# terran-project/terran

Hardware: AMD Instinct MI355X
Metric: frames/sec 1080p detect+embed+pose (higher is better)
Workload: dtype f16x3: operands x = hi + lo (two IEEE halfs, 22 bits), 3 f16 MFMAs per product, f32 accumulate; float32-grade results; 1 GPU; BASELINE configs[4]: 1080p detect+embed+pose; Detection(short_side=416) + Recognition(top-2) + Estimation(short_side=184); 32 frames per GPU per step resident in HBM; random-init weights; precision=f16x3, frames_per_gpu_step=32, faces_per_frame=2, resident_batch_reused=True, batches_in_flight_per_gpu=2

## Files before the change

### include/terran_amd.h

```cpp
#ifndef TERRAN_AMD_H
#define TERRAN_AMD_H

#include <stddef.h>
#include <stdint.h>

#ifdef __cplusplus
extern "C" {
#endif

#define TA_OK 0
#define TA_E_INVALID (-1)
#define TA_E_DEVICE (-2)
#define TA_E_CAPACITY (-3)
#define TA_E_OVERFLOW (-4)
#define TA_E_RANGE (-5)

#define TA_MODEL_RETINAFACE 1
#define TA_MODEL_ARCFACE 2
#define TA_MODEL_OPENPOSE 3

typedef struct ta_ctx ta_ctx;
typedef struct ta_model ta_model;
typedef struct ta_frames ta_frames;

// ... 260 lines not shown

int ta_jpeg_encode_header(int h, int w, int quality, int subsampling, uint8_t* out, size_t capacity, size_t* size);
int ta_jpeg_encode(ta_ctx* ctx, const ta_frames* frames, int quality, int subsampling, const uint8_t** out,
                   size_t* sizes);
int ta_jpeg_encode_last_stats(const ta_ctx* ctx, double* ms, int64_t* counts);
int ta_jpeg_encode_opt(ta_ctx* ctx, const ta_frames* frames, int quality, int subsampling, int optimize,
                       const uint8_t** out, size_t* sizes);
int ta_jpeg_optimal_table(const int64_t* freq, uint8_t* bits, uint8_t* vals, int* nvals);
int ta_jpeg_encode_last_opt_stats(const ta_ctx* ctx, double* ms);

int ta_model_load(ta_ctx* ctx, int kind, const void* blob, size_t bytes, ta_model** out);
int ta_program_check(int kind, const void* blob, size_t bytes, char* msg, size_t msg_capacity);
void ta_model_free(ta_model* m);
int ta_model_kind(const ta_model* m);

int ta_model_forward_frames(ta_model* m, const ta_frames* frames);
int ta_model_forward_crops(ta_model* m, const uint8_t* crops_nchw_bgr, int n);
int ta_model_tensor_shape(ta_model* m, int tensor, int* n, int* c, int* h, int* w);
int ta_model_read_tensor(ta_model* m, int tensor, int ch_off, int ch, float* dst_nchw);

int ta_model_tensor_unscale(const ta_model* m, int tensor, float* out, int capacity);
int ta_model_debug_amax(ta_model* m, int enable, float* out, int capacity);
int ta_model_graph_probe(ta_model* m, int reps, double* out_ms);

int ta_retinaface_run(ta_model* m, const ta_frames* frames, float score_thr, float nms_thr,
                      int capacity, int32_t* counts, float* boxes, float* landmarks, float* scores,
                      int32_t* required);
int ta_retinaface_postprocess(ta_ctx* ctx, const float* const heads[9], int n, int h, int w,
                              float score_thr, float nms_thr, int capacity, int32_t* counts,
                              float* boxes, float* landmarks, float* scores, int32_t* required);

int ta_arcface_embed_crops(ta_model* m, const uint8_t* crops_nchw_bgr, int n, int normalize, float* out);
int ta_arcface_embed_faces(ta_model* m, const ta_frames* frames, const int32_t* frame_index,
                           const double* inv_affine, int n, int normalize, float* out,
                           uint8_t* crops_out);
int ta_arcface_embed_faces_multi(ta_model* m, const ta_frames* const* frames, int n_sources, const int32_t* source_index,
                                 const int32_t* frame_index, const double* inv_affine, int n, int normalize,
                                 float* out, uint8_t* crops_out);
int ta_cosine_distance(ta_ctx* ctx, const float* a, int na, const float* b, int nb, int dim, float* out);

typedef struct ta_gallery ta_gallery;
int ta_gallery_create(ta_ctx* ctx, int dim, int64_t reserve_rows, ta_gallery** out);
void ta_gallery_free(ta_gallery* g);
int ta_gallery_add(ta_gallery* g, const float* rows, const int32_t* ids, int64_t n, int normalize);
int ta_gallery_remove(ta_gallery* g, const int32_t* ids, int n, int64_t* removed);
int ta_gallery_clear(ta_gallery* g);
int ta_gallery_size(const ta_gallery* g, int64_t* rows, int64_t* live);
int ta_gallery_download(const ta_gallery* g, float* rows_out, int32_t* ids_out);
int ta_gallery_search(ta_gallery* g, const float* queries, int nq, int k, int normalize, int32_t* out_row, int32_t* out_id,
                      float* out_dist);
int ta_gallery_cluster(ta_gallery* g, float threshold, int min_samples, int32_t* labels_out, int32_t* degree_out,
                       int32_t* n_clusters, int32_t* rounds);

int ta_openpose_run(ta_model* m, const ta_frames* frames, double scale, int capacity,
                    int32_t* counts, int32_t* keypoints, double* scores, int32_t* required);
int ta_openpose_group(ta_ctx* ctx, const float* pafs, const float* heatmaps, int n, int h, int w,
                      double scale, int capacity, int32_t* counts, int32_t* keypoints,
                      double* scores, int32_t* required);
int ta_openpose_last_stats(const ta_ctx* ctx, int64_t* peaks, int64_t* connections);

int ta_openpose_debug_read(ta_ctx* ctx, int n, int cap_peaks, int32_t* peak_counts, int32_t* peaks_yx,
                           float* peak_scores, int cap_conn, int32_t* conn_counts, int32_t* conn_ij,
                           float* conn_scores);
int ta_openpose_debug_capacity(ta_ctx* ctx, int n, int32_t* peak_capacity);

int ta_bicubic_x8(ta_ctx* ctx, const float* maps, int n, int c, int h, int w, float* out);

#define TA_CONV_AUTO 0
#define TA_CONV_GENERIC 1
#define TA_CONV_PIPE64 2
#define TA_CONV_PIPE128 3
#define TA_CONV_SPLIT_2x2 4
#define TA_CONV_SPLIT_2x2_P8 5
#define TA_CONV_SPLIT_2x4 6
#define TA_CONV_SPLIT_1x4 7
#define TA_CONV_WIN_2x2 8
#define TA_CONV_WIN_2x4 9
#define TA_CONV_WIN_1x4 10
#define TA_CONV_SPLIT_1x4_W2 11
#define TA_CONV_SPLIT_2x2_W2 12
int ta_debug_conv_variant(ta_ctx* ctx, int variant);
int ta_debug_range_check(ta_ctx* ctx);
int ta_debug_conv_counts(ta_ctx* ctx, int64_t* counts16, int reset);
int ta_debug_kernel_work(ta_ctx* ctx, char* csv, size_t capacity, int reset);

#ifdef __cplusplus
}
#endif
#endif
```

### terran_amd/csrc/conv_common.h

```cpp
#pragma once
#include <stdio.h>

#include "act_format.h"
#include "ta_internal.h"

#ifdef TA_CONV_TRACE
static __device__ __attribute__((unused)) long long ta_trace_buf[64];
#define TA_STAMP(i)                                                              \
  do {                                                                           \
    if (blockIdx.x == (unsigned)p.trace_block && (threadIdx.x & 63) == 0) ta_trace_buf[(i)] = __builtin_readcyclecounter(); \
  } while (0)
#define TA_TRACE_READER(name)                                                                   \
  extern "C" int name(long long* out, int n) {                                                  \
    return (int)hipMemcpyFromSymbol(out, HIP_SYMBOL(ta_trace_buf), sizeof(long long) * n);      \
  }
#else
#define TA_STAMP(i) do { } while (0)
#define TA_TRACE_READER(name)
#endif

typedef float f32x16 __attribute__((ext_vector_type(16)));
typedef float f32x4 __attribute__((ext_vector_type(4)));
typedef __bf16 bf16x8 __attribute__((ext_vector_type(8)));
typedef _Float16 f16x8 __attribute__((ext_vector_type(8)));

enum { PREC_F32 = 0, PREC_BF16X3 = 1, PREC_BF16 = 2, PREC_F16X3 = 3, PREC_F16 = 4, PREC_F16X2 = 5 };
__host__ __device__ constexpr bool prec_x3(int prec) { return prec == PREC_BF16X3 || prec == PREC_F16X3; }
__host__ __device__ constexpr bool prec_x2(int prec) { return prec == PREC_F16X2; }
__host__ __device__ constexpr bool prec_half(int prec) { return prec == PREC_F16X3 || prec == PREC_F16 || prec == PREC_F16X2; }
__host__ __device__ constexpr int prec_nmma(int prec) { return prec_x3(prec) ? 3 : (prec_x2(prec) ? 2 : 1); }

template <int PREC>
__device__ __forceinline__ f32x16 ta_mfma16(const bf16x8& a, const bf16x8& b, const f32x16& c) {
  if constexpr (prec_half(PREC))
    return __builtin_amdgcn_mfma_f32_32x32x16_f16(__builtin_bit_cast(f16x8, a), __builtin_bit_cast(f16x8, b), c, 0, 0, 0);
  else
    return __builtin_amdgcn_mfma_f32_32x32x16_bf16(a, b, c, 0, 0, 0);
}
template <int PREC>
__device__ __forceinline__ __bf16 ta_to16(float x) {
  if constexpr (prec_half(PREC)) return __builtin_bit_cast(__bf16, (_Float16)x);
  else return (__bf16)x;
}
template <int PREC>
__device__ __forceinline__ float ta_from16(__bf16 h) {
  if constexpr (prec_half(PREC)) return (float)__builtin_bit_cast(_Float16, h);
  else return (float)h;
}

#define LDS_PTR(p) ((__attribute__((address_space(3))) void*)(p))
#define GLB_PTR(p) ((const __attribute__((address_space(1))) void*)(p))

__device__ __forceinline__ void ta_dma16(const char* ubase, unsigned lane_off, const float* lds_dst) {
  const unsigned ldsa = (unsigned)(size_t)LDS_PTR(lds_dst);
  asm volatile("s_mov_b32 m0, %2\n\ts_nop 0\n\tglobal_load_lds_dwordx4 %0, %1" ::"v"(lane_off), "s"(ubase), "s"(ldsa)
               : "memory", "m0");
}

__device__ __forceinline__ int ta_xcd_tile(int n_pt, int xcd, int local) {
  const int base = n_pt >> 3, rem = n_pt & 7;
  if (local >= base + (xcd < rem ? 1 : 0)) return -1;
  return xcd * base + (xcd < rem ? xcd : rem) + local;
}

#define TA_INTERIOR 5
__device__ __forceinline__ int ta_border_class(int y, int x, int Ho, int Wo) {
  const int cy = Ho == 1 ? 3 : (y == 0 ? 0 : (y == Ho - 1 ? 2 : 1));
  const int cx = Wo == 1 ? 3 : (x == 0 ? 0 : (x == Wo - 1 ? 2 : 1));
  return cy * 4 + cx;
}

#define TA_F16_MAX_BITS 0x477FE000u
__device__ __forceinline__ unsigned ta_absbits(float x) { return __float_as_uint(x) & 0x7FFFFFFFu; }
__device__ __forceinline__ unsigned ta_amax4(unsigned m, const f32x4& v) {
  return max(max(m, max(ta_absbits(v[0]), ta_absbits(v[1]))), max(ta_absbits(v[2]), ta_absbits(v[3])));
}
__device__ __forceinline__ void ta_range_report(const ta_conv_launch& p, unsigned amax) {
  if (amax > TA_F16_MAX_BITS) *p.range_flag = 1;
  if (p.amax_index >= 0 && amax) atomicMax((unsigned*)p.range_flag + TA_AMAX_SLOT0 + 2 * p.amax_index, amax);
}
__device__ __forceinline__ float ta_relu(float v) { return v < 0.f ? 0.f : v; }

template <int WM_TILES, int WN_TILES>
__device__ __forceinline__ void conv_epilogue(const ta_conv_launch& p, f32x16 (&acc)[WM_TILES][WN_TILES], int co_tile0,
// ... 55 lines not shown
    if (p.act == TA_ACT_RELU) {
#pragma unroll
      for (int a = 0; a < WM_TILES; ++a)
#pragma unroll
        for (int j = 0; j < 4; ++j)
#pragma unroll
          for (int e = 0; e < 4; ++e) v[a][j][e] = ta_relu(v[a][j][e]);
    } else if (p.act == TA_ACT_PRELU) {
#pragma unroll
      for (int a = 0; a < WM_TILES; ++a)
#pragma unroll
        for (int j = 0; j < 4; ++j)
#pragma unroll
          for (int e = 0; e < 4; ++e) v[a][j][e] = v[a][j][e] > 0.f ? v[a][j][e] : v[a][j][e] * slope[a][j][e];
    }
    if (p.res) {
      const int ry = p.res_up2 ? (y >> 1) : y, rx = p.res_up2 ? (x >> 1) : x;
      const float* rs = p.res + (size_t)img * p.res_img + (size_t)ry * p.res_row + (size_t)rx * p.res_pix + p.res_off0;
      f32x4 r4[WM_TILES][4];
#pragma unroll
      for (int a = 0; a < WM_TILES; ++a)
#pragma unroll
        for (int j = 0; j < 4; ++j) {
          const int co = co_base + a * 32 + 8 * j;
          r4[a][j] = ta_ld4(rs, p.res_ch + (co < co_max ? co : co_max), p.res_fmt);
        }
#pragma unroll
      for (int a = 0; a < WM_TILES; ++a)
#pragma unroll
        for (int j = 0; j < 4; ++j)
#pragma unroll
          for (int e = 0; e < 4; ++e) v[a][j][e] += r4[a][j][e];
    }
    float* o = p.out + (size_t)img * p.out_img + (size_t)y * p.out_row + (size_t)x * p.out_pix + p.out_off0;
    if (pix_ok) {
#pragma unroll
      for (int a = 0; a < WM_TILES; ++a)
#pragma unroll
        for (int j = 0; j < 4; ++j) {
          const int co = co_base + a * 32 + 8 * j;
          if (co < p.cout) {
            ta_st4(o, p.out_ch + co, p.out_fmt, v[a][j]);
            if (p.range_check) amax = ta_amax4(amax, v[a][j]);
          }
        }
    }
    if (p.out2) {
      float* o2 = p.out2 + (size_t)img * p.o2_img + (size_t)y * p.o2_row + (size_t)x * p.o2_pix + p.o2_off0;
      f32x4 sc[WM_TILES][4], sh[WM_TILES][4];
#pragma unroll
      for (int a = 0; a < WM_TILES; ++a)
#pragma unroll
        for (int j = 0; j < 4; ++j) {
          sc[a][j] = *(const f32x4*)(p.scale2 + co_base + a * 32 + 8 * j);
          sh[a][j] = *(const f32x4*)(p.shift2 + co_base + a * 32 + 8 * j);
        }
      if (pix_ok) {
#pragma unroll
        for (int a = 0; a < WM_TILES; ++a)
#pragma unroll
          for (int j = 0; j < 4; ++j) {
            const int co = co_base + a * 32 + 8 * j;
            f32x4 z;
#pragma unroll
            for (int e = 0; e < 4; ++e) z[e] = v[a][j][e] * sc[a][j][e] + sh[a][j][e];
            if (co < p.cout) {
              ta_st4(o2, p.o2_ch + co, p.o2_fmt, z);
              if (p.range_check) amax = ta_amax4(amax, z);
            }
          }
      }
    }
  }
  ta_range_report(p, amax);
}

struct ta_k_walk {
  int cb, kx, ky, b_off, a_slab;
  int cblocks, kw, kh, pix_bytes, row_bytes;
  __device__ __forceinline__ ta_k_walk(const ta_conv_launch& p, int s0) {
    cblocks = p.k_cblocks;
    kw = p.k_w;
    kh = p.k_h;
    pix_bytes = p.in_pix * 4;
    row_bytes = p.in_row * 4;
    if (s0 == 0) {
      cb = kx = ky = b_off = a_slab = 0;
      return;
    }
    const int taps = kw * kh;
    cb = s0 / taps;
    const int tap = s0 - cb * taps;
    ky = tap / kw;
    kx = tap - ky * kw;
    b_off = cb * 128 + kx * pix_bytes + ky * row_bytes;
    a_slab = tap * cblocks + cb;
  }
  __device__ __forceinline__ void advance() {
    ++kx;
    b_off += pix_bytes;
    a_slab += cblocks;
    if (kx == kw) {
      kx = 0;
      b_off += row_bytes - kw * pix_bytes;
      if (++ky == kh) {
        ky = 0;
        ++cb;
        b_off += 128 - kh * row_bytes;
        a_slab = cb;
      }
    }
  }
};

__device__ __forceinline__ int ta_div_r(int t, int d, float rd, int fast) {
  if (!fast) return t / d;
  int q = (int)((float)t * rd);
  const int r = t - q * d;
  if (r < 0) --q;
  else if (r >= d) ++q;
  return q;
}

struct ta_pixel_walk {
  int img0, y0, x0, Wo, Ho;
  float rWo, rHo;
  __device__ __forceinline__ ta_pixel_walk(const ta_conv_launch& p, int pt0, int HoWo) {
    Wo = p.Wo;
    Ho = p.Ho;
    if (p.fast_div) {
      img0 = ta_div_r(pt0, HoWo, p.r_HoWo, 1);
      const int rem = pt0 - img0 * HoWo;
      y0 = ta_div_r(rem, Wo, p.r_Wo, 1);
      x0 = rem - y0 * Wo;
      rWo = p.r_Wo;
      rHo = p.r_Ho;
      return;
    }
    img0 = pt0 / HoWo;
    const int rem = pt0 - img0 * HoWo;
    y0 = rem / p.Wo;
    x0 = rem - y0 * p.Wo;
    rWo = 1.0f / (float)p.Wo;
    rHo = 1.0f / (float)p.Ho;
  }
  static __device__ __forceinline__ void divmod(int t, int d, float rd, int& q, int& r) {
    q = (int)((float)t * rd);
    r = t - q * d;
    if (r < 0) {
      --q;
      r += d;
    } else if (r >= d) {
      ++q;
      r -= d;
    }
  }
  __device__ __forceinline__ void at(int d, int& img, int& y, int& x) const {
    int qy, qi;
    divmod(x0 + d, Wo, rWo, qy, x);
    divmod(y0 + qy, Ho, rHo, qi, y);
    img = img0 + qi;
  }
};

struct ta_f32x8 {
  f32x4 a, b;
};
__device__ __forceinline__ ta_f32x8 ta_ld8(const float* pix, int ch, int fmt) {
  ta_f32x8 r;
  if (fmt == TA_FMT_F32) {
    r.a = *(const f32x4*)(pix + ch);
    r.b = *(const f32x4*)(pix + ch + 4);
    return r;
  }
  if (fmt == TA_FMT_F16) {
    const uint4 w = *(const uint4*)((const char*)pix + 2 * ch);
    float v[8];
    ta_unpack2<true>(w.x, v[0], v[1]);
    ta_unpack2<true>(w.y, v[2], v[3]);
    ta_unpack2<true>(w.z, v[4], v[5]);
    ta_unpack2<true>(w.w, v[6], v[7]);
    r.a = f32x4{v[0], v[1], v[2], v[3]};
    r.b = f32x4{v[4], v[5], v[6], v[7]};
    return r;
  }
  const char* q = (const char*)pix + ta_split_chan(ch);
  const uint4 h = *(const uint4*)q, l = *(const uint4*)(q + 64);
  const unsigned hw[4] = {h.x, h.y, h.z, h.w}, lw[4] = {l.x, l.y, l.z, l.w};
  float v[8];
#pragma unroll
  for (int i = 0; i < 4; ++i) {
    float h0, h1, l0, l1;
    if (fmt == TA_FMT_SPLIT16) {
      ta_unpack2<true>(hw[i], h0, h1);
      ta_unpack2<true>(lw[i], l0, l1);
    } else {
// ... 387 lines not shown
        const int c = ((wm * WM_TILES + a) * 32 + 8 * j + 4 * (lane >> 5)) >> 2;
        *(f32x4*)(lds + (row * NCH + (c ^ (row & (NCH - 1)))) * 4) =
            f32x4{acc[a][b][4 * j], acc[a][b][4 * j + 1], acc[a][b][4 * j + 2], acc[a][b][4 * j + 3]};
      }
  }
  __syncthreads();
  if (tid == 0) TA_STAMP(22);
  conv_epilogue_drain<BN, BM, 256>(p, lds, ct0, pt0, tid, HoWo, 0);
}

template <int WM_TILES, int WN_TILES, int PREC>
__device__ __forceinline__ void conv_slab_mma(const float* st, f32x16 (&acc)[WM_TILES][WN_TILES], int a_row0, int b_row0, int fsw,
                                              int fcb, int lane) {
  if constexpr (PREC == PREC_F32) {
#pragma unroll
    for (int g = 0; g < 4; ++g) {
      const int pc = ((fcb + g) ^ fsw) * 4;
      f32x4 av[WM_TILES], bv[WN_TILES];
#pragma unroll
      for (int a = 0; a < WM_TILES; ++a) av[a] = *(const f32x4*)(st + (a_row0 + a * 32) * 32 + pc);
#pragma unroll
      for (int b = 0; b < WN_TILES; ++b) bv[b] = *(const f32x4*)(st + (b_row0 + b * 32) * 32 + pc);
#pragma unroll
      for (int e = 0; e < 4; ++e)
#pragma unroll
        for (int a = 0; a < WM_TILES; ++a)
#pragma unroll
          for (int b = 0; b < WN_TILES; ++b)
            acc[a][b] = __builtin_amdgcn_mfma_f32_32x32x2f32(av[a][e], bv[b][e], acc[a][b], 0, 0, 0);
    }
  } else {
    const int kg = lane >> 5;
#pragma unroll
    for (int t = 0; t < 2; ++t) {
      bf16x8 ah[WM_TILES], al[WM_TILES], bh[WN_TILES], bl[WN_TILES];
#pragma unroll
      for (int a = 0; a < WM_TILES; ++a) {
        ah[a] = *(const bf16x8*)(st + (a_row0 + a * 32) * 32 + ((2 * kg + t) ^ fsw) * 4);
        if constexpr (prec_x3(PREC) || prec_x2(PREC)) al[a] = *(const bf16x8*)(st + (a_row0 + a * 32) * 32 + ((4 + 2 * kg + t) ^ fsw) * 4);
      }
#pragma unroll
      for (int b = 0; b < WN_TILES; ++b) {
        const f32x4 x0 = *(const f32x4*)(st + (b_row0 + b * 32) * 32 + ((fcb + 2 * t) ^ fsw) * 4);
        const f32x4 x1 = *(const f32x4*)(st + (b_row0 + b * 32) * 32 + ((fcb + 2 * t + 1) ^ fsw) * 4);
#pragma unroll
        for (int e = 0; e < 4; ++e) {
          const __bf16 h0 = ta_to16<PREC>(x0[e]), h1 = ta_to16<PREC>(x1[e]);
          bh[b][e] = h0;
          bh[b][4 + e] = h1;
          if constexpr (prec_x3(PREC)) {
            bl[b][e] = ta_to16<PREC>(x0[e] - ta_from16<PREC>(h0));
            bl[b][4 + e] = ta_to16<PREC>(x1[e] - ta_from16<PREC>(h1));
          }
        }
      }
      if constexpr (prec_x3(PREC) || prec_x2(PREC)) {
#pragma unroll
        for (int a = 0; a < WM_TILES; ++a)
#pragma unroll
          for (int b = 0; b < WN_TILES; ++b)
            acc[a][b] = ta_mfma16<PREC>(al[a], bh[b], acc[a][b]);
      }
      if constexpr (prec_x3(PREC)) {
#pragma unroll
        for (int a = 0; a < WM_TILES; ++a)
#pragma unroll
          for (int b = 0; b < WN_TILES; ++b)
            acc[a][b] = ta_mfma16<PREC>(ah[a], bl[b], acc[a][b]);
      }
#pragma unroll
      for (int a = 0; a < WM_TILES; ++a)
#pragma unroll
        for (int b = 0; b < WN_TILES; ++b)
          acc[a][b] = ta_mfma16<PREC>(ah[a], bh[b], acc[a][b]);
    }
  }
}

struct ta_tile_grid {
  int n_ct, n_pt, groups;
  ta_tile_grid(const ta_conv_launch& p, int BN, int BM) : n_ct(p.coutp / BN), n_pt((p.M + BM - 1) / BM), groups(((n_pt + 7) / 8) * n_ct) {}
};

#define TA_NOTE_KERNEL(ctx, ...)                                    \
  do {                                                              \
    static char _name[80];                                          \
    if (!_name[0]) snprintf(_name, sizeof(_name), __VA_ARGS__);     \
    (ctx)->note_kernel(_name);                                      \
  } while (0)
```

### terran_amd/csrc/conv_igemm.hip

```cpp
#include <string.h>

#include "conv_common.h"

static bool is_split_variant(int v) {
  return v == TA_CV_SPLIT_2x2 || v == TA_CV_SPLIT_2x2_P8 || v == TA_CV_SPLIT_2x4 || v == TA_CV_SPLIT_1x4 || v == TA_CV_SPLIT_1x4_W2 || v == TA_CV_SPLIT_2x2_W2;
}

static bool variant_eligible(int v, const ta_conv_launch& p) {
  const bool split_in = p.in_fmt == ta_split_fmt_of(p.prec);
  const bool deep = p.uniform_k && (p.n_slabs >= 2 || p.prec == PREC_F16);
  const bool staged = ((p.out_ch | p.res_ch | p.o2_ch) & 7) == 0 && (p.cout & 3) == 0;
  switch (v) {
    case TA_CV_GENERIC: return p.in_fmt == TA_FMT_F32 && !p.group_cout;
    case TA_CV_PIPE64: return deep && staged && p.coutp % 64 == 0 && !p.group_cout && (p.in_fmt == TA_FMT_F32 || (split_in && p.prec != PREC_F16));
    case TA_CV_PIPE128: return deep && staged && p.coutp % 128 == 0 && !p.group_cout && p.in_fmt == TA_FMT_F32;
    case TA_CV_SPLIT_2x2:
    case TA_CV_SPLIT_2x2_P8:
    case TA_CV_SPLIT_2x4: return deep && split_in && staged && p.coutp % 128 == 0;
    case TA_CV_SPLIT_1x4: return deep && split_in && staged && p.coutp % 64 == 0 && (!p.group_cout || p.group_cout % 64 == 0);
    case TA_CV_SPLIT_2x2_W2: return deep && split_in && staged && p.coutp % 128 == 0 && p.k_split <= 1;
    case TA_CV_SPLIT_1x4_W2: return deep && split_in && staged && p.coutp % 64 == 0 && (!p.group_cout || p.group_cout % 64 == 0) && p.k_split <= 1;
    case TA_CV_WIN_2x2:
    case TA_CV_WIN_2x4:
    case TA_CV_WIN_1x4: {
      const bool base = deep && split_in && staged && (p.prec == PREC_F16X3 || p.prec == PREC_F16X2) && p.stride == 1 && !p.pool && p.k_split <= 1 &&
                        p.k_w * p.k_h >= 4 && p.n_slabs == p.k_w * p.k_h * p.k_cblocks;
      if (!base) return false;
      if (v == TA_CV_WIN_1x4) return p.coutp % 64 == 0 && (!p.group_cout || p.group_cout % 64 == 0) && ta_win_patch_rows(p, 256) <= TA_WIN_PR_1x4;
      if (p.coutp % 128) return false;
      return v == TA_CV_WIN_2x2 ? ta_win_patch_rows(p, 128) <= TA_WIN_PR_2x2 : ta_win_patch_rows(p, 256) <= TA_WIN_PR_2x4;
    }
  }
  return false;
}

static int choose_variant_streamed(const ta_conv_launch& p);
static int choose_variant(const ta_conv_launch& p) {
  const int v = choose_variant_streamed(p);
  const int w = v == TA_CV_SPLIT_2x2 ? TA_CV_WIN_2x2 : (v == TA_CV_SPLIT_2x4 ? TA_CV_WIN_2x4 : (v == TA_CV_SPLIT_1x4 ? TA_CV_WIN_1x4 : 0));
  return (w && variant_eligible(w, p)) ? w : v;
}
static int choose_variant_streamed(const ta_conv_launch& p) {
  if (p.uniform_k && (p.n_slabs >= 2 || p.prec == PREC_F16)) {
    if (variant_eligible(TA_CV_SPLIT_2x2, p)) {
      if (p.prec != PREC_F32 && p.k_split == 1) {
        const int n_ct = p.coutp / 128;
        const int t1 = ((p.M + 127) / 128) * n_ct, t2 = ((p.M + 255) / 256) * n_ct;
        const int r1 = (t1 + 255) / 256, r2 = (t2 + 255) / 256;
        if (r2 * 184 < r1 * 100) return TA_CV_SPLIT_2x4;
      }
      return TA_CV_SPLIT_2x2;
    }
    if (variant_eligible(TA_CV_SPLIT_1x4, p)) {
      constexpr int W2_SLABS = 18, W2_TILES = 1024;
      if (p.prec != PREC_F32 && p.n_slabs <= W2_SLABS && (p.M + 255) / 256 * (p.coutp / 64) >= W2_TILES && variant_eligible(TA_CV_SPLIT_1x4_W2, p))
        return TA_CV_SPLIT_1x4_W2;
      return TA_CV_SPLIT_1x4;
    }
    if (variant_eligible(TA_CV_PIPE64, p)) return TA_CV_PIPE64;
  }
  return TA_CV_GENERIC;
}

static int launch_variant(ta_ctx* ctx, int v, const ta_conv_launch& p) {
  switch (v) {
    case TA_CV_GENERIC:
    case TA_CV_PIPE64:
    case TA_CV_PIPE128: return ta_launch_conv_sym(ctx, v, p);
    case TA_CV_SPLIT_2x2:
    case TA_CV_SPLIT_2x2_P8:
    case TA_CV_SPLIT_2x4:
    case TA_CV_SPLIT_1x4:
    case TA_CV_SPLIT_1x4_W2:
    case TA_CV_SPLIT_2x2_W2:
    case TA_CV_WIN_2x2:
    case TA_CV_WIN_2x4:
    case TA_CV_WIN_1x4: return ta_launch_conv_split(ctx, v, p);
  }
  return ta_fail(ctx, TA_E_INVALID, "conv: unknown kernel variant %d", v);
}

int ta_launch_conv(ta_ctx* ctx, const ta_conv_launch& p_in, double flops) {
  if (p_in.M <= 0) return TA_OK;
  ta_conv_launch p = p_in;
#ifdef TA_CONV_TRACE
  p.trace_block = ctx->conv_trace_block;
#endif
  if (p.k_split < 1 || !p.partial) p.k_split = 1;
  if (p.coutp % 32 != 0 || p.cout % 4 != 0) return ta_fail(ctx, TA_E_INVALID, "conv: bad cout padding");
  if (p.prec != PREC_F32 && p.prec != PREC_BF16X3 && p.prec != PREC_BF16 && p.prec != PREC_F16X3 && p.prec != PREC_F16 && p.prec != PREC_F16X2)
    return ta_fail(ctx, TA_E_INVALID, "conv: unknown precision mode %d", p.prec);
  if (p.in_fmt != TA_FMT_F32 && p.in_fmt != ta_split_fmt_of(p.prec))
    return ta_fail(ctx, TA_E_INVALID, "conv: input tensor format %d does not belong to precision mode %d", p.in_fmt, p.prec);
  p.range_flag = ctx->range_flag;
  int v = p.variant;
  if (v != TA_CV_AUTO) {
    if (!variant_eligible(v, p))
      return ta_fail(ctx, TA_E_INVALID, "conv: forced kernel variant %d cannot run this layer (cin-uniform %d, slabs %d, coutp %d, "
                     "input format %d, groups %d)", v, p.uniform_k, p.n_slabs, p.coutp, p.in_fmt, p.group_cout ? 1 : 0);
  } else {
    const bool prefer = ctx->conv_force && variant_eligible(ctx->conv_force, p) && (!p.pool || is_split_variant(ctx->conv_force));
    v = prefer ? ctx->conv_force : choose_variant(p);
    if (!variant_eligible(v, p)) return ta_fail(ctx, TA_E_INVALID, "conv: pre-split input reached a kernel that cannot read it");
  }
  const bool is_split = is_split_variant(v);
  if (!is_split || v == TA_CV_SPLIT_1x4_W2 || v == TA_CV_SPLIT_2x2_W2) p.k_split = 1;
  if (p.pool) {
    if (!is_split || p.res || p.out2 || (p.out_ch & 7) || (p.M & 3) || (p.act != TA_ACT_RELU && p.act != TA_ACT_NONE))
      return ta_fail(ctx, TA_E_INVALID, "conv: the fused max-pool needs the split-role kernel and a plain epilogue (variant %d)", v);
    p.k_split = 1;
  }
  ctx->conv_counts[v] += 1;
  ctx->cur_flops = flops;
  ta_prof_scope scope(ctx, 0, flops);
  return launch_variant(ctx, v, p);
}

extern "C" {

int ta_debug_conv_variant(ta_ctx* ctx, int variant) {
  if (!ctx || variant < 0 || variant >= TA_CV_COUNT) return TA_E_INVALID;
  ctx->conv_force = variant;
  return TA_OK;
}

int ta_debug_kernel_work(ta_ctx* ctx, char* csv, size_t capacity, int reset) {
  if (!ctx || (!csv && capacity)) return TA_E_INVALID;
  std::string out;
  for (const auto& kv : ctx->kernel_work) {
    char line[200];
    const auto t = ctx->kernel_ms.find(kv.first);
    snprintf(line, sizeof(line), "%s;%lld;%.6e;%.6f\n", kv.first.c_str(), (long long)kv.second.first, kv.second.second,
             t == ctx->kernel_ms.end() ? 0.0 : t->second);
    out += line;
  }
  if (reset) {
    ta_drain_profile(ctx);
    ctx->kernel_work.clear();
    ctx->kernel_ms.clear();
  }
  if (out.size() + 1 > capacity) return ta_fail(ctx, TA_E_CAPACITY, "kernel_work: %zu bytes needed", out.size() + 1);
  memcpy(csv, out.c_str(), out.size() + 1);
  return TA_OK;
}

int ta_debug_conv_counts(ta_ctx* ctx, int64_t* counts16, int reset) {
  if (!ctx) return TA_E_INVALID;
  for (int i = 0; i < TA_CV_COUNT; ++i) {
    if (counts16) counts16[i] = ctx->conv_counts[i];
    if (reset) ctx->conv_counts[i] = 0;
  }
  return TA_OK;
}

}
```

### terran_amd/csrc/conv_split_kernels.h

```cpp
#pragma once
#include "conv_common.h"

__device__ __forceinline__ void split_acc_clear(f32x16 (&acc)[2][2]) {
#pragma unroll
  for (int a = 0; a < 2; ++a)
#pragma unroll
    for (int b = 0; b < 2; ++b)
#pragma unroll
      for (int r = 0; r < 16; ++r) acc[a][b][r] = 0.f;
}

template <int PREC>
__device__ __forceinline__ void split_mma16(f32x16 (&acc)[2][2], const bf16x8 (&ah)[2], const bf16x8 (&al)[2], const bf16x8 (&bh)[2],
                                            const bf16x8 (&bl)[2]) {
  if constexpr (prec_x3(PREC) || prec_x2(PREC)) {
#pragma unroll
    for (int a = 0; a < 2; ++a)
#pragma unroll
      for (int b = 0; b < 2; ++b) acc[a][b] = ta_mfma16<PREC>(al[a], bh[b], acc[a][b]);
  }
  if constexpr (prec_x3(PREC)) {
#pragma unroll
    for (int a = 0; a < 2; ++a)
#pragma unroll
      for (int b = 0; b < 2; ++b) acc[a][b] = ta_mfma16<PREC>(ah[a], bl[b], acc[a][b]);
  }
  if constexpr (PREC == PREC_F16) {
#pragma unroll
    for (int a = 0; a < 2; ++a)
#pragma unroll
      for (int b = 0; b < 2; ++b) acc[a][b] = ta_mfma16<PREC>(al[a], bl[b], acc[a][b]);
  }
#pragma unroll
  for (int a = 0; a < 2; ++a)
#pragma unroll
    for (int b = 0; b < 2; ++b) acc[a][b] = ta_mfma16<PREC>(ah[a], bh[b], acc[a][b]);
}

template <int NREAD, int NMMA>
__device__ __forceinline__ void split_pin() {
#pragma unroll
  for (int i = 0; i < NREAD; ++i) {
    __builtin_amdgcn_sched_group_barrier(0x100, 1, 0);
    __builtin_amdgcn_sched_group_barrier(0x008, 1, 0);
  }
  __builtin_amdgcn_sched_group_barrier(0x008, NMMA - NREAD, 0);
}


template <int CM, int CN, int NP, int PREC, int STAGES>
__global__ __launch_bounds__(64 * (CM * CN + NP), STAGES == 2 ? 4 : (CM * CN + NP) / 4) void conv_igemm_split(const ta_conv_launch p) {
  static_assert(NP == 4 || NP == 8, "4 or 8 producer waves");
  static_assert(STAGES == 3 || (STAGES == 2 && CM * CN == 4 && NP == 4), "3-stage ring, or the 2-stage two-workgroups-per-CU variant of the 8-wave tiles");
  static_assert(CM * CN == 4 || CM * CN == 8, "consumer grid: 1x4 (64 cout x 256 px), 2x2 (128 x 128) or 2x4 (128 x 256)");
  constexpr int NC = CM * CN;
  constexpr int BN = CM * 64, BM = CN * 64;
  constexpr int NI = (BN + BM) / 8 / NP;
  constexpr int QA = BN / 8 / NP;
  constexpr int STAGE = (BN + BM) * 32;
  extern __shared__ __attribute__((aligned(16))) float lds[];

  const int tid = threadIdx.x;
  const int lane = tid & 63;
  const int wave = __builtin_amdgcn_readfirstlane(tid >> 6);
  if (wave == 0) TA_STAMP(0);
  if (wave == NC) TA_STAMP(8);

  const int n_ct = p.coutp / BN;
  const int n_pt = (p.M + BM - 1) / BM;
  const int tile_blocks = (((n_pt + 7) >> 3) * n_ct) << 3;
  const int ks = p.k_split > 1 ? ta_div_r(blockIdx.x, tile_blocks, p.r_tile_blocks, p.fast_div) : 0;
  const int bid = blockIdx.x - ks * tile_blocks;
  const int grp = bid >> 3, xcd = bid & 7;
  const int gq = ta_div_r(grp, n_ct, p.r_nct, p.fast_div);
  const int pt = ta_xcd_tile(n_pt, xcd, gq);
  if (pt < 0) return;
  const int ct0 = (grp - gq * n_ct) * BN;
  const int pt0 = pt * BM;
  const int HoWo = p.Ho * p.Wo;
  int s_begin = 0, S = p.n_slabs;
  if (p.k_split > 1) {
    s_begin = (int)(((long long)ks * p.n_slabs) / p.k_split);
    S = (int)(((long long)(ks + 1) * p.n_slabs) / p.k_split) - s_begin;
  }

  if (wave >= NC) {
    const int pw = wave - NC;
    const int pchunk = lane & 7;
    const int lchunk = pchunk ^ ((4 * (pw & 1) + (lane >> 4)) & 7);
    const char* a_base = (const char*)p.w;
    const size_t a_slab_bytes = (size_t)p.coutp * 128;
    unsigned a_off[QA];
    unsigned b_off[NI - QA];
#pragma unroll
    for (int q = 0; q < QA; ++q) a_off[q] = (unsigned)(((ct0 + (q * NP + pw) * 8 + (lane >> 3)) * 32 + lchunk * 4) * 4);
    ta_k_walk wa(p, s_begin);
    auto issue_a = [&](int, int stage) {
#pragma unroll
      for (int q = 0; q < QA; ++q) ta_dma16(a_base + (size_t)wa.a_slab * a_slab_bytes, a_off[q], lds + stage * STAGE + (q * NP + pw) * 256);
      wa.advance();
    };
    issue_a(0, 0);
    if (S > 1) issue_a(1, 1);
    const int pl = p.pool;
    const ta_pixel_walk walk(p, pl ? pt0 >> 2 : pt0, HoWo);
    const int in_ch = p.in_ch_off + (p.group_cout ? (ct0 / p.group_cout) * p.group_cin : 0);
    const size_t off0 = (size_t)walk.img0 * p.in_img + (size_t)((walk.y0 << pl) * p.stride) * p.in_row +
                        (size_t)((walk.x0 << pl) * p.stride) * p.in_pix + p.in_off0 + in_ch;
    const char* b_base = (const char*)(p.in + off0);
    ta_k_walk wb(p, s_begin);
#pragma unroll
    for (int q = QA; q < NI; ++q) {
      const int d = (q * NP + pw) * 8 + (lane >> 3) - BN;
      int img, y, x;
      const int dd = pt0 + d < p.M ? d : 0;
      walk.at(pl ? dd >> 2 : dd, img, y, x);
      if (pl) {
        y = 2 * y + ((dd >> 1) & 1);
        x = 2 * x + (dd & 1);
      }
      const size_t off = (size_t)img * p.in_img + (size_t)(y * p.stride) * p.in_row + (size_t)(x * p.stride) * p.in_pix +
                         p.in_off0 + in_ch;
      b_off[q - QA] = (unsigned)((off - off0) * 4 + lchunk * 16);
      ta_dma16(b_base + wb.b_off, b_off[q - QA], lds + (q * NP + pw) * 256);
    }
    wb.advance();
    auto issue_b = [&](int stage) {
#pragma unroll
      for (int q = QA; q < NI; ++q) ta_dma16(b_base + wb.b_off, b_off[q - QA], lds + stage * STAGE + (q * NP + pw) * 256);
      wb.advance();
    };
    if (wave == NC) TA_STAMP(9);
    if (S > 1) issue_b(1);
    if (wave == NC) TA_STAMP(10);
    int stage = STAGES == 2 ? 0 : 2;
    if constexpr (STAGES == 2) {
      for (int s = 0; s < S; ++s) {
        if (s == 0 && S > 1) asm volatile("s_waitcnt vmcnt(%0)" ::"n"(NI - QA) : "memory");
        else asm volatile("s_waitcnt vmcnt(0)" ::: "memory");
        __builtin_amdgcn_s_barrier();
        asm volatile("" ::: "memory");
        if (s >= 1 && s + 1 < S) {
          issue_a(s + 1, stage);
          issue_b(stage);
          stage ^= 1;
        }
      }
    } else
    for (int s = 0; s < S; ++s) {
      if (s == 0 && S > 1) asm volatile("s_waitcnt vmcnt(%0)" ::"n"(NI - QA) : "memory");
      else if (s + 1 < S) asm volatile("s_waitcnt vmcnt(%0)" ::"n"(NI) : "memory");
      else asm volatile("s_waitcnt vmcnt(0)" ::: "memory");
      __builtin_amdgcn_s_barrier();
      asm volatile("" ::: "memory");
      if (s + 2 < S) {
        issue_a(s + 2, stage);
        issue_b(stage);
        stage = stage == 2 ? 0 : stage + 1;
      }
    }
    {
      __builtin_amdgcn_s_barrier();
      __builtin_amdgcn_s_barrier();
      asm volatile("" ::: "memory");
      bool done = false;
      if constexpr (PREC != PREC_F32) done = conv_drain_dispatch<BN, BM, 64 * (NC + NP), (PREC == PREC_F16 ? 2 : (prec_half(PREC) ? 1 : 0))>(p, lds, ct0, pt0, tid, HoWo);
      if (!done) conv_epilogue_drain<BN, BM, 64 * (NC + NP)>(p, lds, ct0, pt0, tid, HoWo, ks);
    }
    return;
  }

  const int cm = wave / CN, cn = wave % CN;
  int stage = 0;
  f32x16 acc[2][2];
  split_acc_clear(acc);
  const int frow = lane & 31;
  const int fsw = (frow >> 1) & 7;
  const int kg = lane >> 5;
  const int a_row0 = cm * 64 + frow;
  const int b_row0 = BN + cn * 64 + frow;
  struct Frag {
    bf16x8 ah[2], al[2], bh[2], bl[2];
    f32x4 a32[2][2], b32[2][2];
  };
  const int fcb = kg * 4;
  auto load = [&](Frag& f, const float* st, int t) {
    if constexpr (PREC == PREC_F32) {
#pragma unroll
      for (int g = 0; g < 2; ++g) {
        const int pc = ((fcb + 2 * t + g) ^ fsw) * 4;
#pragma unroll
        for (int a = 0; a < 2; ++a) f.a32[a][g] = *(const f32x4*)(st + (a_row0 + a * 32) * 32 + pc);
#pragma unroll
        for (int b = 0; b < 2; ++b) f.b32[b][g] = *(const f32x4*)(st + (b_row0 + b * 32) * 32 + pc);
      }
      return;
    }
#pragma unroll
    for (int a = 0; a < 2; ++a) {
      f.ah[a] = *(const bf16x8*)(st + (a_row0 + a * 32) * 32 + ((2 * kg + t) ^ fsw) * 4);
      if constexpr (prec_x3(PREC) || prec_x2(PREC) || PREC == PREC_F16) f.al[a] = *(const bf16x8*)(st + (a_row0 + a * 32) * 32 + ((4 + 2 * kg + t) ^ fsw) * 4);
    }
#pragma unroll
    for (int b = 0; b < 2; ++b) {
      f.bh[b] = *(const bf16x8*)(st + (b_row0 + b * 32) * 32 + ((2 * kg + t) ^ fsw) * 4);
      if constexpr (prec_x3(PREC) || PREC == PREC_F16) f.bl[b] = *(const bf16x8*)(st + (b_row0 + b * 32) * 32 + ((4 + 2 * kg + t) ^ fsw) * 4);
    }
  };
  auto mma = [&](const Frag& f) {
    if constexpr (PREC == PREC_F32) {
#pragma unroll
      for (int g = 0; g < 2; ++g)
#pragma unroll
// ... 205 lines not shown
      pb[b] = (unsigned)buf * (unsigned)(PATCH * 4) + row * 128u + ((((unsigned)(2 * kg)) ^ ((row >> 1) & 7u)) << 4);
    }
  };
  auto load = [&](Frag& f, const float* st, int t) {
#pragma unroll
    for (int a = 0; a < 2; ++a) {
      f.ah[a] = *(const bf16x8*)(st + (a_row0 + a * 32) * 32 + ((2 * kg + t) ^ fsw) * 4);
      f.al[a] = *(const bf16x8*)(st + (a_row0 + a * 32) * 32 + ((4 + 2 * kg + t) ^ fsw) * 4);
    }
#pragma unroll
    for (int b = 0; b < 2; ++b) {
      const char* q = (const char*)patch0 + (pb[b] ^ (unsigned)(t << 4));
      f.bh[b] = *(const bf16x8*)q;
      if constexpr (prec_x3(PREC)) f.bl[b] = *(const bf16x8*)((const char*)patch0 + ((pb[b] ^ (unsigned)(t << 4)) ^ 64u));
    }
  };
  auto mma = [&](const Frag& f) { split_mma16<PREC>(acc, f.ah, f.al, f.bh, f.bl); };
  constexpr int NREAD = prec_x3(PREC) ? 8 : 6;
  constexpr int NMMA = prec_x3(PREC) ? 12 : 8;
  int kx = 0, ky = 0, cb = 0, tap_off = 0, stage = 0;
  Frag F0, F1;
  baddr(0, 0);
  if (wave == 0) TA_STAMP(1);
  __builtin_amdgcn_s_barrier();
  asm volatile("" ::: "memory");
  if (wave == 0) TA_STAMP(2);
  load(F0, lds, 0);
  for (int g = 0; g + 1 < S; ++g) {
    const float* st = lds + stage * A_STAGE;
    stage = stage == 2 ? 0 : stage + 1;
    __builtin_amdgcn_sched_barrier(0);
    load(F1, st, 1);
    mma(F0);
    split_pin<NREAD, NMMA>();
    __builtin_amdgcn_sched_barrier(0);
    if (++kx == p.k_w) {
      kx = 0;
      tap_off += wp - p.k_w;
      if (++ky == p.k_h) {
        ky = 0;
        ++cb;
        tap_off = -1;
      }
    }
    ++tap_off;
    asm volatile("s_waitcnt lgkmcnt(0)" ::: "memory");
    baddr(tap_off, cb & 1);
    __builtin_amdgcn_s_barrier();
    asm volatile("" ::: "memory");
    load(F0, lds + stage * A_STAGE, 0);
    mma(F1);
    split_pin<NREAD, NMMA>();
    __builtin_amdgcn_sched_barrier(0);
  }
  load(F1, lds + stage * A_STAGE, 1);
  mma(F0);
  mma(F1);
  if (wave == 0) TA_STAMP(3);
  {
    __builtin_amdgcn_s_barrier();
    asm volatile("" ::: "memory");
    if (wave == 0) TA_STAMP(5);
    conv_epilogue_park<BN>(acc, lds, cm, cn, lane);
    if (wave == 0) TA_STAMP(6);
    asm volatile("s_waitcnt lgkmcnt(0)" ::: "memory");
    __builtin_amdgcn_s_barrier();
    asm volatile("" ::: "memory");
    if (wave == 0) TA_STAMP(7);
    if (!conv_drain_dispatch<BN, BM, 64 * (NC + NP), 1>(p, lds, ct0, pt0, tid, HoWo))
      conv_epilogue_drain<BN, BM, 64 * (NC + NP)>(p, lds, ct0, pt0, tid, HoWo, 0);
  }
  if (wave == 0) TA_STAMP(4);
}

static void split_launch_facts(ta_ctx* ctx, ta_conv_launch& q, const ta_tile_grid& g, int BM, int split_fmt, bool lean_ok) {
  q.r_nct = 1.0f / (float)g.n_ct;
  q.r_tile_blocks = 1.0f / (float)(g.groups * 8);
  q.r_Wo = 1.0f / (float)q.Wo;
  q.r_Ho = 1.0f / (float)q.Ho;
  q.r_HoWo = 1.0f / (float)(q.Ho * q.Wo);
  const long long grid = (long long)g.groups * 8 * q.k_split;
  q.fast_div = (grid < (1 << 24) && (long long)q.M + BM < (1 << 24)) ? 1 : 0;
  const long long n_img = q.Ho * q.Wo > 0 ? ((long long)q.M + q.Ho * q.Wo - 1) / (q.Ho * q.Wo) : 0;
  auto fits = [&](long long img_stride, int off0) { return ((n_img + 1) * img_stride + off0) * 4 < (1LL << 32); };
  bool ok = lean_ok && q.out_fmt == split_fmt && (q.cout & 7) == 0 && ((q.out_ch | q.res_ch | q.o2_ch) & 7) == 0 && fits(q.out_img, q.out_off0);
  if (q.res) ok = ok && q.res_fmt == split_fmt && fits(q.res_img, q.res_off0);
  if (q.out2) ok = ok && q.o2_fmt == split_fmt && fits(q.o2_img, q.o2_off0);
  const bool plain = !q.res && !q.out2;
  ok = ok && (q.pool ? (plain && q.act == TA_ACT_RELU) : (q.bias9 ? (plain && q.act == TA_ACT_PRELU) : (plain || (q.res && q.act == TA_ACT_NONE))));
  q.fast_drain = ok ? 1 : 0;
  if (ok) ctx->conv_counts[TA_CV_COUNT - 1] += 1;
}

template <int CM, int CN, int NP, int PREC, int STAGES>
static int launch_split(ta_ctx* ctx, const ta_conv_launch& p) {
  constexpr int BN = CM * 64, BM = CN * 64;
  const ta_tile_grid g(p, BN, BM);
  const size_t lds_bytes = (size_t)STAGES * (BN + BM) * 32 * sizeof(float);
  auto kern = conv_igemm_split<CM, CN, NP, PREC, STAGES>;
  TA_SET_LDS_ATTR(ctx, kern, lds_bytes);
  ta_conv_launch q = p;
  constexpr int SPLIT_FMT = PREC == PREC_F16 ? TA_FMT_F16 : (prec_half(PREC) ? TA_FMT_SPLIT16 : TA_FMT_SPLIT);
  split_launch_facts(ctx, q, g, BM, SPLIT_FMT, PREC != PREC_F32 && p.k_split == 1);
  TA_NOTE_KERNEL(ctx, "conv_igemm_split<%d,%d,%d,%d,%d>", CM, CN, NP, PREC, STAGES);
  hipLaunchKernelGGL(kern, dim3(g.groups * 8 * p.k_split), dim3(64 * (CM * CN + NP)), lds_bytes, ctx->stream, q);
  TA_HIP(ctx, hipGetLastError());
  return TA_OK;
}

template <int CM, int CN, int PREC, int PR>
static int launch_win(ta_ctx* ctx, const ta_conv_launch& p) {
  constexpr int BN = CM * 64, BM = CN * 64;
  const ta_tile_grid g(p, BN, BM);
  constexpr size_t ring = (size_t)(3 * BN + 2 * PR) * 128, park = (size_t)BM * BN * 4;
  constexpr size_t lds_bytes = ring > park ? ring : park;
  static_assert(lds_bytes <= 160 * 1024, "one workgroup's LDS");
  auto kern = conv_igemm_win<CM, CN, PREC, PR>;
  TA_SET_LDS_ATTR(ctx, kern, lds_bytes);
  ta_conv_launch q = p;
  q.k_split = 1;
  split_launch_facts(ctx, q, g, BM, TA_FMT_SPLIT16, true);
  TA_NOTE_KERNEL(ctx, "conv_igemm_win<%d,%d,%d,%d>", CM, CN, PREC, PR);
  hipLaunchKernelGGL(kern, dim3(g.groups * 8), dim3(64 * (CM * CN + 4)), lds_bytes, ctx->stream, q);
  TA_HIP(ctx, hipGetLastError());
  return TA_OK;
}

template <int PREC>
static int launch_split_variant(ta_ctx* ctx, int v, const ta_conv_launch& p) {
  switch (v) {
    case TA_CV_SPLIT_2x2: return launch_split<2, 2, 4, PREC, 3>(ctx, p);
    case TA_CV_SPLIT_2x2_P8: return launch_split<2, 2, 8, PREC, 3>(ctx, p);
    case TA_CV_SPLIT_2x4: return launch_split<2, 4, 4, PREC, 3>(ctx, p);
    case TA_CV_SPLIT_1x4: return launch_split<1, 4, 4, PREC, 3>(ctx, p);
    case TA_CV_SPLIT_1x4_W2: return launch_split<1, 4, 4, PREC, 2>(ctx, p);
    case TA_CV_SPLIT_2x2_W2: return launch_split<2, 2, 4, PREC, 2>(ctx, p);
    case TA_CV_WIN_2x2:
    case TA_CV_WIN_2x4:
    case TA_CV_WIN_1x4:
      if constexpr (PREC == PREC_F16X3 || PREC == PREC_F16X2) {
        if (v == TA_CV_WIN_2x2) return launch_win<2, 2, PREC, TA_WIN_PR_2x2>(ctx, p);
        if (v == TA_CV_WIN_2x4) return launch_win<2, 4, PREC, TA_WIN_PR_2x4>(ctx, p);
        return launch_win<1, 4, PREC, TA_WIN_PR_1x4>(ctx, p);
      }
      break;
  }
  return ta_fail(ctx, TA_E_INVALID, "conv: unknown kernel variant %d", v);
}
```

### terran_amd/csrc/model_load.hip

```cpp
#include <stdarg.h>
#include <string.h>

#include "act_format.h"
#include "ta_internal.h"

namespace {
struct refusal {
  char* msg;
  size_t cap;
  int operator()(const char* fmt, ...) const {
    if (msg && cap) {
      va_list ap;
      va_start(ap, fmt);
      vsnprintf(msg, cap, fmt, ap);
      va_end(ap);
    }
    return TA_E_INVALID;
  }
};
const int MAX_DIM = 1 << 24;
bool within(int v, int lo, int hi) { return v >= lo && v <= hi; }
}

int ta_program_parse(int kind, const void* blob, size_t bytes, ta_program* out, char* msg, size_t msg_capacity) {
  const refusal no{msg, msg_capacity};
  if (msg && msg_capacity) msg[0] = 0;
  if (!blob || !out) return no("model blob: null pointer");
  if (bytes < sizeof(ta_blob_header)) return no("model blob too small");
  ta_blob_header& h = out->hdr;
  memcpy(&h, blob, sizeof(h));
  if (h.magic != TA_BLOB_MAGIC || h.version != 9) return no("model blob: bad magic/version (this library reads version 9)");
  if (h.kind != kind) return no("model blob is kind %d, expected %d", h.kind, kind);
  if (h.n_tensors <= 0 || h.n_ops <= 0 || h.n_outputs < 0 || h.n_outputs > 16 || h.input_tensor < 0 ||
      h.input_tensor >= h.n_tensors)
    return no("model blob: bad counts");
  auto inside = [&](int64_t off, int64_t count, size_t each) {
    return off >= 0 && count >= 0 && (uint64_t)off <= bytes && (uint64_t)count <= (bytes - (size_t)off) / each;
  };
  if (!inside(h.tensors_off, h.n_tensors, sizeof(ta_tensor_desc))) return no("model blob: truncated (tensor table)");
  if (!inside(h.ops_off, h.n_ops, sizeof(ta_op_desc))) return no("model blob: truncated (op table)");
  if (!inside(h.weights_off, h.weights_bytes, 1)) return no("model blob: truncated (weights)");
  const int T = h.n_tensors;
  std::vector<ta_tensor_desc>& td = out->tdesc;
  std::vector<ta_op_desc>& ops = out->ops;
  td.resize(T);
  ops.resize(h.n_ops);
  memcpy(td.data(), (const char*)blob + h.tensors_off, T * sizeof(ta_tensor_desc));
  memcpy(ops.data(), (const char*)blob + h.ops_off, h.n_ops * sizeof(ta_op_desc));
  auto bad_w = [&](int64_t off, size_t need) { return off >= 0 && (uint64_t)off + need > (uint64_t)h.weights_bytes; };

  for (int t = 0; t < T; ++t) {
    const ta_tensor_desc& d = td[t];
    if (!within(d.channels, 1, MAX_DIM) || !within(d.halo, 0, 1024) || !within(d.alias_of, -2, T - 1) || d.alias_of == t)
      return no("model blob: malformed tensor %d", t);
    if ((d.fmt != TA_FMT_F32 && d.channels % 32) || (d.fmt == TA_FMT_F16 && d.channels % 64) || d.fmt < 0 || d.fmt > TA_FMT_F16)
      return no("model blob: tensor %d: format %d with %d channels", t, d.fmt, d.channels);
    if (d.unscale_off >= 0 && (t == h.input_tensor || (d.unscale_off & 3) || bad_w(d.unscale_off, (size_t)d.channels * sizeof(float))))
      return no("model blob: inconsistent activation scales (tensor %d)", t);
  }
  for (int i = 0; i < h.n_outputs; ++i)
    if (!within(h.outputs[i], 0, T - 1)) return no("model blob: output %d is tensor %d, out of range", i, h.outputs[i]);

  std::vector<char> set(T, 0);
  set[h.input_tensor] = 1;
  auto view_ready = [&](int id) {
    const int src = td[id].alias_of;
    if (src >= 0 && !set[id]) set[id] = set[src];
    return src < 0 || set[id];
  };
  std::vector<int> writer_lane(T, 0), reader_lanes(T, 0);

  for (int oi = 0; oi < h.n_ops; ++oi) {
    const ta_op_desc& op = ops[oi];
    auto bad_t = [&](int t) { return t < 0 || t >= T; };
    const char* why = nullptr;
    auto need = [&](bool ok, const char* what) {
      if (!ok && !why) why = what;
    };
    need(!bad_t(op.in) && !bad_t(op.out) && (op.res < 0 || !bad_t(op.res)) && (op.out2 < 0 || !bad_t(op.out2)), "tensor index out of range");
    need(within(op.kh, 1, 64) && within(op.kw, 1, 64) && within(op.stride, 1, 64) && within(op.pad, 0, 64) && within(op.cin, 0, MAX_DIM) &&
             within(op.cout, 0, MAX_DIM) && within(op.coutp, 0, MAX_DIM) && within(op.n_slabs, 0, MAX_DIM) && within(op.groups, 0, 1 << 16) &&
             within(op.in_ch_off, 0, MAX_DIM) && within(op.out_ch_off, 0, MAX_DIM) && within(op.res_ch_off, 0, MAX_DIM) &&
             within(op.out2_ch_off, 0, MAX_DIM),
         "field out of range");
    if (why) return no("model blob: malformed op %d: %s", oi, why);
    const size_t row = (size_t)op.coutp * 4, image = (size_t)op.n_slabs * op.coutp * 128;
    const bool wus_ok = !bad_w(op.bias_off, row) && op.wus_off == op.bias_off + 4 * (int64_t)op.coutp && !bad_w(op.wus_off, row);
    if (op.type == TA_OP_CONV) {
      need(op.w_off >= 0 && op.bias_off >= 0, "no weights or no bias");
      need(op.cin % 4 == 0 && op.cout % 4 == 0 && op.coutp % 32 == 0 && op.n_slabs > 0, "channel counts or K slabs");
      need(op.prec >= 0 && op.prec <= 5, "arithmetic mode");
      need(!bad_w(op.w_off, image), "w_off past the weight region");
      need(!bad_w(op.bias_off, row), "bias_off past the weight region");
      need(!bad_w(op.prelu_off, row), "prelu_off past the weight region");
      need(!bad_w(op.scale2_off, row), "scale2_off past the weight region");
      need(!bad_w(op.shift2_off, row), "shift2_off past the weight region");
      need(wus_ok, "wus_off is not the [coutp] floats behind the bias");
      need(op.act != TA_ACT_PRELU || op.prelu_off >= 0, "PReLU without slopes");
      need(op.out2 < 0 || (op.scale2_off >= 0 && op.shift2_off >= 0), "second output without its affine");
      need(!ta_op_border_bias(op) || !(op.out2 >= 0 || op.scale2_off < 0 || op.kh != 3 || op.kw != 3 || op.stride != 1 || op.pad != 1 ||
                                       op.pool || bad_w(op.scale2_off, 16 * row)),
           "border-bias table on a conv that is not a plain 3x3, stride 1, pad 1");
    } else if (op.type == TA_OP_RFSTEM) {
      need(op.w_off >= 0 && (op.cout == 16 || op.cout == 32), "front op without weights or with another width than 16 / 32");
      need(!bad_w(op.w_off, (op.cout == 32 ? 448 + 704 : 448) * 4), "w_off past the weight region");
    } else if (op.type == TA_OP_DWPW) {
      need(op.w_off >= 0 && op.bias_off >= 0 && op.scale2_off >= 0 && op.shift2_off >= 0, "no weights or no bias");
      need(op.cin % 4 == 0 && op.cout % 4 == 0 && op.coutp % 32 == 0 && op.n_slabs > 0 && (int64_t)op.n_slabs * 32 >= op.cin && op.stride <= 2,
           "channel counts, K slabs or stride");
      need(op.prec == 0 || op.prec == 3, "arithmetic mode");
      need(!bad_w(op.w_off, image), "w_off past the weight region");
      need(!bad_w(op.bias_off, row), "bias_off past the weight region");
      need(!bad_w(op.scale2_off, (size_t)op.cin * 36), "scale2_off past the weight region");
      need(!bad_w(op.shift2_off, (size_t)op.cin * 4), "shift2_off past the weight region");
      need(wus_ok, "wus_off is not the [coutp] floats behind the bias");
    } else if (op.type == TA_OP_DWCONV) {
      need(op.w_off >= 0 && op.bias_off >= 0 && op.cin % 4 == 0 && op.kh == 3 && op.kw == 3, "no weights, no bias, or not 3x3");
      need(!bad_w(op.w_off, (size_t)op.cin * 36), "w_off past the weight region");
      need(!bad_w(op.bias_off, (size_t)op.cin * 4), "bias_off past the weight region");
    } else if (op.type != TA_OP_MAXPOOL && op.type != TA_OP_COPYCH) {
      return no("model blob: unknown op type %d (op %d)", op.type, oi);
    }
    if (why) return no("model blob: malformed op %d: %s", oi, why);

    const ta_tensor_desc &ti = td[op.in], &to = td[op.out];
    if (!view_ready(op.in)) return no("model blob: alias tensor %d used before its source %d (op %d)", op.in, ti.alias_of, oi);
    if (!set[op.in]) return no("model blob: op %d reads unset tensor %d", oi, op.in);
    if (op.type != TA_OP_CONV && (ti.fmt == TA_FMT_F16 || to.fmt == TA_FMT_F16))
      return no("model blob: op %d: only convs read and write half-float tensors", oi);
    if ((op.type == TA_OP_CONV || op.type == TA_OP_DWCONV) && ti.halo < op.pad)
      return no("model blob: op %d needs halo %d, tensor has %d", oi, op.pad, ti.halo);
    if (op.type == TA_OP_CONV) {
      const ta_k_geometry kg = ta_conv_k_geometry(op, ti.fmt);
      if (op.groups > 1 && !(kg.uniform && op.n_slabs >= 2 && op.cout % op.groups == 0 && (op.cout / op.groups) % 128 == 0 && op.cout == op.coutp &&
                             op.in_ch_off % 32 == 0 && op.in_ch_off + (int64_t)op.groups * op.cin <= ti.channels && ti.fmt == ta_split_fmt_of(op.prec)))
        return no("model blob: op %d: unsupported grouped convolution", oi);
      if (op.pool && (op.out2 >= 0 || op.res >= 0 || op.groups > 1 || op.cin % 32 || op.coutp % 64))
        return no("model blob: op %d: unsupported conv + max-pool fusion", oi);
      if (ti.fmt == TA_FMT_F16 && (!kg.uniform || op.in_ch_off || op.groups > 1 || op.prec != 4))
        return no("model blob: op %d: a half-float tensor feeds whole-tensor convs of the f16 mode only", oi);
      if (ti.fmt != TA_FMT_F16 && (int64_t)op.kh * op.kw * (op.cin / 4) > (int64_t)op.n_slabs * 8)
        return no("model blob: op %d has too few K slabs", oi);
    } else if (op.type == TA_OP_DWCONV) {
      if (op.in_ch_off || op.out_ch_off) return no("model blob: op %d: depthwise conv on a channel slice is not supported", oi);
      if (ti.unscale_off >= 0 || to.unscale_off >= 0) return no("model blob: inconsistent activation scales (op %d)", oi);
    } else if (op.type == TA_OP_RFSTEM) {
      if (oi != 0 || op.in != h.input_tensor || ti.alias_of != -2)
        return no("model blob: the RetinaFace front op must be op 0 on a shape-only input tensor (op %d)", oi);
    } else if (op.type == TA_OP_DWPW) {
      if (ti.halo < 1) return no("model blob: op %d (dw+pw) needs an input halo", oi);
      if (ti.fmt != TA_FMT_F32 || op.in_ch_off || op.cin > ti.channels) return no("model blob: op %d: unsupported dw+pw block", oi);
    }
    set[op.out] = 1;
    if (op.out2 >= 0) set[op.out2] = 1;

    const int lane = ta_op_lane(op);
    bool shared = lane == 3 || (lane && (op.type != TA_OP_CONV || ta_op_packed_ksplit(op) > 1 || op.pool));
    for (int t : {op.in, op.res}) {
      if (t < 0) continue;
      if (writer_lane[t] && writer_lane[t] != lane) shared = true;
      reader_lanes[t] |= 1 << lane;
    }
    for (int t : {op.out, op.out2}) {
      if (t < 0) continue;
      if (reader_lanes[t] & ~(1 << lane)) shared = true;
      if (writer_lane[t] && writer_lane[t] != lane) shared = true;
      if (lane) writer_lane[t] = lane;
      else if (reader_lanes[t] >> 1) shared = true;
    }
    if (shared) return no("model blob: an op lane (side stream) shares tensors with ops outside it (op %d)", oi);
  }
  for (int t = 0; t < T; ++t)
    if (!view_ready(t)) return no("model blob: alias tensor %d used before its source %d", t, td[t].alias_of);
  return TA_OK;
}

extern "C" {

int ta_program_check(int kind, const void* blob, size_t bytes, char* msg, size_t msg_capacity) {
  ta_program p;
  return ta_program_parse(kind, blob, bytes, &p, msg, msg_capacity);
}

int ta_model_load(ta_ctx* ctx, int kind, const void* blob, size_t bytes, ta_model** out) {
  ta_enter(ctx);
  if (!ctx || !blob || !out) return TA_E_INVALID;
  *out = nullptr;
  std::unique_ptr<ta_model> m(new ta_model());
  char why[256];
  if (ta_program_parse(kind, blob, bytes, m.get(), why, sizeof(why)) != TA_OK) return ta_fail(ctx, TA_E_INVALID, "%s", why);
  const ta_blob_header& h = m->hdr;
  const char* weights = (const char*)blob + h.weights_off;
  m->ctx = ctx;
  m->kind = kind;
  m->unscale_host.resize(h.n_tensors);
  for (int t = 0; t < h.n_tensors; ++t)
    if (m->tdesc[t].unscale_off >= 0) {
      const float* v = (const float*)(weights + m->tdesc[t].unscale_off);
      m->unscale_host[t].assign(v, v + m->tdesc[t].channels);
    }
  m->tensor_read.assign(h.n_tensors, 0);
  for (auto& op : m->ops) {
    m->tensor_read[op.in] = 1;
    if (op.res >= 0) m->tensor_read[op.res] = 1;
    if ((op.type == TA_OP_CONV || op.type == TA_OP_DWPW) && (op.prec == 3 || op.prec == 4 || op.prec == 5)) m->has_half_ops = true;
  }
  for (int t = 0; t < h.n_tensors; ++t) {
    const int src = m->tdesc[t].alias_of;
// ... 34 lines not shown
```

### terran_amd/csrc/model_plan.hip

```cpp
#include <algorithm>

#include "act_format.h"
#include "ta_internal.h"

#define TA_MAX_PLANS 4
#define TA_MAX_PLAN_BYTES ((size_t)96 << 30)

static int conv_out(int in, int k, int stride, int pad) { return (in + 2 * pad - k) / stride + 1; }

static void activate(ta_model* m, ta_plan* pl, int n_run) {
  m->active = pl;
  pl->last_use = ++m->use_counter;
  m->run_n = n_run;
}

static int plan_capacity(int kind, int n) {
  if (kind != TA_MODEL_ARCFACE) return n;
  if (n <= 8) return 8;
  if (n <= 32) return 32;
  return (n + 63) / 64 * 64;
}

static int infer_shapes(const ta_model* m, int h, int w, std::vector<ta_tensor>& ts, std::vector<bool>& set) {
  ta_ctx* ctx = m->ctx;
// ... 21 lines not shown
    set[id] = true;
    return TA_OK;
  };

  for (const ta_op_desc& op : m->ops) {
    TA_TRY(resolve_alias(op.in));
    const ta_tensor& ti = ts[op.in];
    switch (op.type) {
      case TA_OP_CONV:
      case TA_OP_DWCONV: {
        const int oh = conv_out(ti.h, op.kh, op.stride, op.pad), ow = conv_out(ti.w, op.kw, op.stride, op.pad);
        if (op.type == TA_OP_CONV && op.pool) {
          TA_TRY(set_out(op.out, oh / 2, ow / 2));
          break;
        }
        TA_TRY(set_out(op.out, oh, ow));
        if (op.type == TA_OP_CONV && op.out2 >= 0) TA_TRY(set_out(op.out2, oh, ow));
        break;
      }
      case TA_OP_MAXPOOL:
        TA_TRY(set_out(op.out, ti.h / 2, ti.w / 2));
        break;
      case TA_OP_RFSTEM:
        if (op.cout == 32)
          TA_TRY(set_out(op.out, ((ti.h + 1) / 2 + 1) / 2, ((ti.w + 1) / 2 + 1) / 2));
        else
          TA_TRY(set_out(op.out, (ti.h + 1) / 2, (ti.w + 1) / 2));
        break;
      case TA_OP_DWPW:
        TA_TRY(set_out(op.out, conv_out(ti.h, 3, op.stride, 1), conv_out(ti.w, 3, op.stride, 1)));
        break;
      case TA_OP_COPYCH:
        TA_TRY(set_out(op.out, ti.h, ti.w));
        break;
    }
  }
  for (size_t i = 0; i < ts.size(); ++i) TA_TRY(resolve_alias((int)i));
  return TA_OK;
}

int ta_model_plan(ta_model* m, int n_run, int h, int w) {
  ta_ctx* ctx = m->ctx;
  if (n_run <= 0 || h <= 0 || w <= 0) return ta_fail(ctx, TA_E_INVALID, "plan: bad input shape %dx%dx%d", n_run, h, w);
  const int n = plan_capacity(m->kind, n_run);
  auto fits = [&](const ta_plan* pl) { return pl && pl->n == n && pl->h == h && pl->w == w; };
  if (fits(m->active)) {
    activate(m, m->active, n_run);
    return TA_OK;
  }
  for (auto& pl : m->plans)
    if (fits(pl.get())) {
      activate(m, pl.get(), n_run);
      return TA_OK;
    }
  TA_HIP(ctx, hipStreamSynchronize(ctx->stream));
  for (;;) {
    size_t bytes = 0;
    for (auto& pl : m->plans) bytes += pl->arena_bytes;
    if (m->plans.size() < TA_MAX_PLANS && bytes <= TA_MAX_PLAN_BYTES) break;
    if (m->plans.empty()) break;
    size_t lru = 0;
    for (size_t i = 1; i < m->plans.size(); ++i)
      if (m->plans[i]->last_use < m->plans[lru]->last_use) lru = i;
    if (m->plans[lru].get() == m->active) m->active = nullptr;
    m->plans.erase(m->plans.begin() + lru);
  }
  std::unique_ptr<ta_plan> np(new ta_plan());
  np->n = n;
  np->h = h;
  np->w = w;

  const int T = m->hdr.n_tensors;
  std::vector<ta_tensor> ts(T);
  std::vector<bool> set(T, false);
  for (int i = 0; i < T; ++i) {
    ts[i].c = m->tdesc[i].channels;
    ts[i].halo = m->tdesc[i].halo;
    ts[i].fmt = m->tdesc[i].fmt;
    if (m->tdesc[i].unscale_off >= 0) {
      ts[i].unscale_dev = (const float*)(m->weights_dev + m->tdesc[i].unscale_off);
      ts[i].unscale_host = m->unscale_host[i].data();
    }
    ts[i].n = n;
  }
  TA_TRY(infer_shapes(m, h, w, ts, set));

  size_t total = 0;
  std::vector<size_t> offs(T, 0);
  for (int i = 0; i < T; ++i) {
    if (!set[i] || !ts[i].owns) continue;
    const size_t bytes = ts[i].elems() * sizeof(float);
    if (bytes >= ((size_t)1 << 32)) return ta_fail(ctx, TA_E_INVALID, "plan: tensor %d exceeds 4 GiB; split the batch", i);
    offs[i] = total;
    total += (bytes + 255) & ~(size_t)255;
  }
  size_t ws_bytes = 0;
  for (const ta_op_desc& op : m->ops) {
    if (op.type != TA_OP_CONV) continue;
    const int M = ts[op.out].n * ts[op.out].h * ts[op.out].w;
    const int ks = ta_op_ksplit(op, ts[op.in].fmt);
    if (ks > 1) ws_bytes = std::max(ws_bytes, (size_t)ks * M * op.coutp * sizeof(float));
  }
  const size_t ws_off = total;
  total += (ws_bytes + 255) & ~(size_t)255;
  hipError_t e = hipMalloc((void**)&np->arena, total ? total : 256);
  if (e != hipSuccess) {
    np->arena = nullptr;
    return ta_fail(ctx, TA_E_DEVICE, "plan: hipMalloc(%zu) failed: %s", total, hipGetErrorString(e));
  }
  np->arena_bytes = total;
  TA_HIP(ctx, hipMemsetAsync(np->arena, 0, total ? total : 256, ctx->stream));
  for (int i = 0; i < T; ++i)
    if (set[i] && ts[i].owns) ts[i].dev = (float*)(np->arena + offs[i]);
  for (int i = 0; i < T; ++i)
    if (set[i] && !ts[i].owns) ts[i].dev = m->tdesc[i].alias_of >= 0 ? ts[m->tdesc[i].alias_of].dev : nullptr;
  np->splitk_ws = ws_bytes ? (float*)(np->arena + ws_off) : nullptr;

  std::vector<int32_t> ktab;
  np->ktab_off.assign(m->ops.size(), 0);
  for (size_t oi = 0; oi < m->ops.size(); ++oi) {
    const ta_op_desc& op = m->ops[oi];
    if (op.type != TA_OP_CONV) continue;
    const ta_tensor& ti = ts[op.in];
    np->ktab_off[oi] = ktab.size();
    if (ti.fmt == TA_FMT_F16) continue;
    const int cpt = op.cin / 4;
    const int nq = op.kh * op.kw * cpt;
    for (int q = 0; q < op.n_slabs * 8; ++q) {
      int32_t off = 0;
      if (q < nq) {
        const int tap = q / cpt, ch = (q % cpt) * 4;
        const int ky = tap / op.kw, kx = tap % op.kw;
        off = (int32_t)((((size_t)ky * ti.wp() + kx) * ti.c + op.in_ch_off + ch) * sizeof(float));
      }
      ktab.push_back(off);
    }
  }
  if (!ktab.empty()) {
    TA_HIP(ctx, hipMalloc((void**)&np->ktab_dev, ktab.size() * sizeof(int32_t)));
    TA_HIP(ctx, hipMemcpy(np->ktab_dev, ktab.data(), ktab.size() * sizeof(int32_t), hipMemcpyHostToDevice));
  }
  TA_HIP(ctx, hipStreamSynchronize(ctx->stream));
  np->tensors.swap(ts);
  m->plans.push_back(std::move(np));
  activate(m, m->plans.back().get(), n_run);
  return TA_OK;
}
```

### terran_amd/csrc/model_run.hip

```cpp
#include <stdlib.h>
#include <string.h>

#include <algorithm>
#include <chrono>

#include "act_format.h"
#include "ta_internal.h"

static int conv_out(int in, int k, int stride, int pad) { return (in + 2 * pad - k) / stride + 1; }

static const float* wptr(const ta_model* m, int64_t off) { return off < 0 ? nullptr : (const float*)(m->weights_dev + off); }

static void put(const ta_strides& s, int& img, int& row, int& pix, int& off0) { img = s.img, row = s.row, pix = s.pix, off0 = s.off0; }

static void print_op_profile(ta_model* m, std::vector<hipEvent_t>& ev) {
  (void)hipStreamSynchronize(m->ctx->stream);
  double tot_ms = 0, tot_fl = 0;
  for (size_t oi = 0; oi < m->ops.size(); ++oi) {
    const ta_op_desc& op = m->ops[oi];
    const ta_tensor& to = m->tensor(op.out);
    float ms = 0.f;
    (void)hipEventElapsedTime(&ms, ev[2 * oi], ev[2 * oi + 1]);
    const ta_tensor& ti = m->tensor(op.in);
    const double M = op.type == TA_OP_CONV && op.pool
// ... 40 lines not shown
  const ta_plan& pl = *m->active;
  for (size_t oi = 0; oi < m->ops.size(); ++oi) {
    const ta_op_desc& op = m->ops[oi];
    const ta_tensor& ti = m->tensor(op.in);
    const ta_tensor& to = m->tensor(op.out);
    const int lane = lanes_on ? ta_op_lane(op) : 0;
    ctx->stream = lanes.main;
    if (lane) {
      const int li = lane - 1;
      if (!ctx->side_stream[li]) {
        TA_HIP(ctx, hipStreamCreateWithFlags(&ctx->side_stream[li], hipStreamNonBlocking));
        TA_HIP(ctx, hipEventCreateWithFlags(&ctx->side_fork[li], hipEventDisableTiming));
        TA_HIP(ctx, hipEventCreateWithFlags(&ctx->side_join[li], hipEventDisableTiming));
      }
      if (!lanes.started[li]) {
        TA_HIP(ctx, hipEventRecord(ctx->side_fork[li], lanes.main));
        TA_HIP(ctx, hipStreamWaitEvent(ctx->side_stream[li], ctx->side_fork[li], 0));
        lanes.started[li] = true;
      }
      ctx->stream = ctx->side_stream[li];
    }
    struct evp_t {
      hipEvent_t e;
      hipStream_t s;
      bool on;
      ~evp_t() { if (on) (void)hipEventRecord(e, s); }
    } evp{prof_ops ? ev[2 * oi + 1] : nullptr, ctx->stream, prof_ops};
    if (prof_ops) (void)hipEventRecord(ev[2 * oi], ctx->stream);
    switch (op.type) {
      case TA_OP_CONV: {
        ta_conv_launch p;
        memset(&p, 0, sizeof(p));
        p.in = ti.dev;
        p.w = wptr(m, op.w_off);
        p.ktab = pl.ktab_dev + pl.ktab_off[oi];
        p.bias = wptr(m, op.bias_off);
        p.prelu = wptr(m, op.prelu_off);
        p.out = to.dev;
        p.M = m->run_n * to.h * to.w;
        p.Ho = to.h;
        p.Wo = to.w;
        p.n_slabs = op.n_slabs;
        p.coutp = op.coutp;
        p.cout = op.cout;
        p.act = op.act;
        p.stride = op.stride;
        p.prec = op.prec;
        const ta_k_geometry kg = ta_conv_k_geometry(op, ti.fmt);
        p.uniform_k = kg.uniform;
        p.k_cblocks = kg.cblocks;
        p.k_w = op.kw;
        p.k_h = op.kh;
        p.in_ch_off = op.in_ch_off;
        put(ta_tensor_strides(ti, op.pad, false), p.in_img, p.in_row, p.in_pix, p.in_off0);
        p.win_wp = ti.wp();
        p.win_img = ti.hp() * ti.wp();
        put(ta_tensor_strides(to, 0, false), p.out_img, p.out_row, p.out_pix, p.out_off0);
        p.out_ch = op.out_ch_off;
        p.out_fmt = to.fmt;
        p.in_fmt = ti.fmt;
        if (op.res >= 0) {
          const ta_tensor& tr = m->tensor(op.res);
          p.res = tr.dev;
          put(ta_tensor_strides(tr, 0, false), p.res_img, p.res_row, p.res_pix, p.res_off0);
          p.res_ch = op.res_ch_off;
          p.res_fmt = tr.fmt;
          p.res_up2 = op.res_up2;
        }
        if (op.out2 >= 0) {
          const ta_tensor& t2 = m->tensor(op.out2);
          p.out2 = t2.dev;
          p.scale2 = wptr(m, op.scale2_off);
          p.shift2 = wptr(m, op.shift2_off);
          put(ta_tensor_strides(t2, 0, false), p.o2_img, p.o2_row, p.o2_pix, p.o2_off0);
          p.o2_ch = op.out2_ch_off;
          p.o2_fmt = t2.fmt;
        }
        if (op.groups > 1) {
          p.group_cout = op.cout / op.groups;
          p.group_cin = op.cin;
        }
        p.variant = ta_op_forced_variant(op);
        if (ta_op_border_bias(op)) p.bias9 = wptr(m, op.scale2_off);
        p.range_check = (m->has_half_ops && (m->tensor_read[op.out] || (op.out2 >= 0 && m->tensor_read[op.out2]))) ? 1 : 0;
        p.amax_index = (m->amax_on && oi < TA_AMAX_OPS) ? (int)oi : -1;
        double flops = 2.0 * op.macs_per_pixel * (double)p.M;
        if (op.pool) {
          p.pool = 1;
          p.M = m->run_n * to.h * to.w * 4;
          flops = 2.0 * op.macs_per_pixel * (double)m->run_n * conv_out(ti.h, op.kh, op.stride, op.pad) *
                  conv_out(ti.w, op.kw, op.stride, op.pad);
        }
        p.k_split = pl.splitk_ws ? ta_op_ksplit(op, ti.fmt) : 1;
        p.partial = pl.splitk_ws;
        if (lane) p.k_split = 1;
        TA_TRY(ta_launch_conv(ctx, p, flops));
        break;
      }
      case TA_OP_RFSTEM:
        TA_TRY(ta_launch_rfstem(ctx, m->input_u8, m->run_n, ti.h, ti.w, (const float*)m->weights_host_small.data(),
                                op.cout == 32 ? wptr(m, op.w_off) + 448 : nullptr, to));
        break;
      case TA_OP_DWPW: {
        ta_conv_launch p;
        memset(&p, 0, sizeof(p));
        p.in = ti.dev;
        p.w = wptr(m, op.w_off);
        p.bias = wptr(m, op.bias_off);
        p.dw_w = wptr(m, op.scale2_off);
        p.dw_bias = wptr(m, op.shift2_off);
        p.dw_c = op.cin;
        p.dw_stride = op.stride;
        p.out = to.dev;
        p.M = m->run_n * to.h * to.w;
        p.Ho = to.h;
        p.Wo = to.w;
        p.n_slabs = op.n_slabs;
        p.coutp = op.coutp;
        p.cout = op.cout;
        p.act = op.act;
        p.stride = 1;
        p.prec = op.prec;
        p.range_check = (m->has_half_ops && m->tensor_read[op.out]) ? 1 : 0;
        p.amax_index = (m->amax_on && oi < TA_AMAX_OPS) ? (int)oi : -1;
        put(ta_tensor_strides(ti, 1, true), p.in_img, p.in_row, p.in_pix, p.in_off0);
        p.in_fmt = ti.fmt;
        put(ta_tensor_strides(to, 0, true), p.out_img, p.out_row, p.out_pix, p.out_off0);
        p.out_ch = op.out_ch_off;
        p.out_fmt = to.fmt;
        TA_TRY(ta_launch_dwpw(ctx, p, 2.0 * op.macs_per_pixel * (double)p.M));
        break;
      }
      case TA_OP_DWCONV: {
        ta_dw_launch p;
        memset(&p, 0, sizeof(p));
        p.in = ti.dev;
        p.w = wptr(m, op.w_off);
        p.bias = wptr(m, op.bias_off);
        p.out = to.dev;
        p.N = m->run_n;
        p.Ho = to.h;
        p.Wo = to.w;
        p.C = op.cin;
        p.stride = op.stride;
        p.relu = op.act == TA_ACT_RELU;
        put(ta_tensor_strides(ti, op.pad, true), p.in_img, p.in_row, p.in_pix, p.in_off0);
        p.in_fmt = ti.fmt;
        put(ta_tensor_strides(to, 0, true), p.out_img, p.out_row, p.out_pix, p.out_off0);
        p.out_fmt = to.fmt;
        TA_TRY(ta_launch_dwconv(ctx, p));
        break;
      }
      case TA_OP_MAXPOOL:
        TA_TRY(ta_launch_maxpool(ctx, ti, to, m->run_n));
        break;
      case TA_OP_COPYCH:
        TA_TRY(ta_launch_copych(ctx, ti, op.in_ch_off, to, op.out_ch_off, op.cin, m->run_n));
        break;
    }
  }
  return TA_OK;
}

extern "C" {

int ta_model_graph_probe(ta_model* m, int reps, double* out_ms) {
// ... 169 lines not shown
```

### terran_amd/csrc/ta_internal.h

```cpp
#pragma once
#include <hip/hip_runtime.h>
#include <stdint.h>
#include <stdio.h>
#include <atomic>
#include <map>
#include <memory>
#include <mutex>
#include <string>
#include <vector>

#include "../../include/terran_amd.h"

#define TA_BLOB_MAGIC 0x314D4154u

enum {
  TA_OP_CONV = 1,
  TA_OP_DWCONV = 2,
  TA_OP_MAXPOOL = 3,
  TA_OP_COPYCH = 4,
  TA_OP_RFSTEM = 5,
  TA_OP_DWPW = 6
};
enum { TA_ACT_NONE = 0, TA_ACT_RELU = 1, TA_ACT_PRELU = 2 };

struct ta_blob_header {
  uint32_t magic;
  uint32_t version;
  int32_t kind;
  int32_t n_tensors;
  int32_t n_ops;
  int32_t input_tensor;
  int32_t n_outputs;
  int32_t outputs[16];
  int64_t tensors_off, ops_off, weights_off, weights_bytes;
};

struct ta_tensor_desc {
  int32_t channels;
  int32_t halo;
  int32_t alias_of;
  int32_t fmt;
  int32_t unscale_off;
};

struct ta_op_desc {
  int32_t type;
  int32_t in, out;
  int32_t in_ch_off, cin;
  int32_t out_ch_off, cout;
  int32_t coutp;
  int32_t kh, kw, stride, pad;
  int32_t act;
  int32_t res, res_ch_off, res_up2;
  int32_t out2, out2_ch_off;
  int32_t n_slabs;
  int32_t prec;
  int32_t groups;
  int32_t variant;
  int32_t pool;
  int32_t wscale_log2;
  int64_t w_off, bias_off, prelu_off, scale2_off, shift2_off;
  int64_t wus_off;
  double macs_per_pixel;
};

static inline int ta_op_forced_variant(const ta_op_desc& op) { return op.variant & 255; }
static inline int ta_op_packed_ksplit(const ta_op_desc& op) { return (op.variant >> 8) & 255; }
static inline bool ta_op_border_bias(const ta_op_desc& op) { return (op.variant >> 16) & 1; }
static inline int ta_op_lane(const ta_op_desc& op) { return (op.variant >> 17) & 3; }

static_assert(sizeof(ta_blob_header) == 128 && sizeof(ta_tensor_desc) == 20 && sizeof(ta_op_desc) == 152,
              "blob layout is shared with terran_amd/pack.py (HEADER_DT / TENSOR_DT / OP_DT)");

struct ta_prof_class {
  double ms = 0;
  int64_t launches = 0;
  double work = 0;
};

struct ta_pending_event {
  hipEvent_t a, b;
  int klass;
  const std::string* kernel;
};

struct ta_ctx {
  int device = -1;
  hipStream_t stream = nullptr;
  std::string err;
  bool profiling = false;
  ta_prof_class prof[4];
  std::vector<ta_pending_event> pending;
  std::vector<hipEvent_t> event_pool;
  hipEvent_t t0 = nullptr, t1 = nullptr;
  void* scratch = nullptr;
  size_t scratch_bytes = 0;
  void* pinned = nullptr;
  size_t pinned_bytes = 0;
  std::mutex frame_cache_mu;
  std::vector<std::pair<size_t, void*>> frame_cache;
  size_t frame_cache_bytes = 0;
  int64_t pose_peaks = 0, pose_connections = 0;
  double jpeg_ms[4] = {0, 0, 0, 0};
  int64_t jpeg_counts[4] = {0, 0, 0, 0};
  double jpeg_enc_ms[8] = {0, 0, 0, 0, 0, 0, 0, 0};
  int64_t jpeg_enc_counts[4] = {0, 0, 0, 0};
  double jpeg_enc_opt_ms[2] = {0, 0};
  void* jpeg_enc_dev = nullptr;
  size_t jpeg_enc_dev_bytes = 0;
  uint8_t* jpeg_enc_out = nullptr;
  size_t jpeg_enc_out_bytes = 0;
  void* yuv_in = nullptr;
  size_t yuv_in_bytes = 0;
  float* pose_wphase = nullptr;
  struct {
    int n = 0, maxp = 0;
    const int *peak_cnt = nullptr, *peak_yx = nullptr, *conn_cnt = nullptr, *conn_ij = nullptr;
    const float *peak_sc = nullptr, *conn_sc = nullptr;
    struct over_t {
      int img, maxp;
      void* mem;
      const int *peak_cnt, *peak_yx, *conn_cnt, *conn_ij;
      const float *peak_sc, *conn_sc;
    };
    std::vector<over_t> over;
  } pose_dbg;
  hipStream_t side_stream[2] = {nullptr, nullptr};
  hipEvent_t side_fork[2] = {nullptr, nullptr}, side_join[2] = {nullptr, nullptr};
  int conv_force = 0;
#ifdef TA_CONV_TRACE
  int conv_trace_block = 0;
#endif
  int64_t conv_counts[16] = {0};
  int* range_flag = nullptr;
  int* range_flag_host = nullptr;
  const void* amax_owner = nullptr;
  double cur_flops = 0;
  std::map<std::string, std::pair<int64_t, double>> kernel_work;
  std::map<std::string, double> kernel_ms;
  const std::string* cur_kernel = nullptr;
  void note_kernel(const char* name) {
    auto it = kernel_work.try_emplace(name, 0, 0.0).first;
    it->second.first += 1;
    it->second.second += cur_flops;
    cur_kernel = &it->first;
  }
};
void ta_pose_free_big(ta_ctx* ctx);
#define TA_AMAX_SLOT0 16
#define TA_AMAX_OPS 4096
int ta_range_enqueue(ta_ctx* ctx);
int ta_range_check(ta_ctx* ctx);
int ta_range_finish(ta_ctx* ctx, int rc);

enum {
  TA_CV_AUTO = 0,
  TA_CV_GENERIC = 1,
  TA_CV_PIPE64 = 2,
  TA_CV_PIPE128 = 3,
  TA_CV_SPLIT_2x2 = 4,
  TA_CV_SPLIT_2x2_P8 = 5,
  TA_CV_SPLIT_2x4 = 6,
  TA_CV_SPLIT_1x4 = 7,
  TA_CV_WIN_2x2 = 8,
  TA_CV_WIN_2x4 = 9,
  TA_CV_WIN_1x4 = 10,
  TA_CV_SPLIT_1x4_W2 = 11,
  TA_CV_SPLIT_2x2_W2 = 12,
  TA_CV_COUNT = 16
};

#define TA_SET_LDS_ATTR(ctx, kern, bytes)                                                                         \
  do {                                                                                                            \
    static std::atomic<unsigned long long> _done{0};                                                              \
    const unsigned long long _bit = 1ull << ((ctx)->device & 63);                                                 \
    if (!(_done.load(std::memory_order_acquire) & _bit)) {                                                        \
      TA_HIP(ctx, hipFuncSetAttribute((const void*)(kern), hipFuncAttributeMaxDynamicSharedMemorySize, (int)(bytes))); \
      _done.fetch_or(_bit, std::memory_order_release);                                                            \
    }                                                                                                             \
  } while (0)

int ta_fail(ta_ctx* ctx, int code, const char* fmt, ...);
static inline void ta_enter(const ta_ctx* ctx) {
  if (ctx) (void)hipSetDevice(ctx->device);
}
int ta_scratch(ta_ctx* ctx, size_t bytes, void** out);
int ta_pinned(ta_ctx* ctx, size_t bytes, void** out);

#define TA_HIP(ctx, expr)                                                                      \
  do {                                                                                         \
    hipError_t _e = (expr);                                                                    \
    if (_e != hipSuccess)                                                                      \
      return ta_fail((ctx), TA_E_DEVICE, "%s failed: %s (%s:%d)", #expr, hipGetErrorString(_e), \
                     __FILE__, __LINE__);                                                      \
  } while (0)

#define TA_TRY(expr)            \
  do {                          \
    int _r = (expr);            \
    if (_r != TA_OK) return _r; \
  } while (0)

struct ta_prof_scope {
  ta_ctx* ctx;
  int klass;
  double work;
  hipEvent_t a = nullptr, b = nullptr;
  ta_prof_scope(ta_ctx* c, int k, double w);
  ~ta_prof_scope();
};

void ta_drain_profile(ta_ctx* ctx);

struct ta_frames {
  ta_ctx* ctx;
  int n, h, w;
  uint8_t* dev;
  size_t cap = 0;
};
int ta_frames_alloc_uninit(ta_ctx* ctx, int n, int h, int w, ta_frames** out);
void ta_disc_rows(int a, int b, std::vector<int2>& tab);

static inline bool ta_fmt_is_half(int fmt) { return fmt == 3; }

struct ta_tensor {
  float* dev = nullptr;
  int n = 0, h = 0, w = 0, c = 0, halo = 0, fmt = 0;
  const float* unscale_dev = nullptr;
  const float* unscale_host = nullptr;
  bool owns = true;
  int hp() const { return h + 2 * halo; }
  int wp() const { return w + 2 * halo; }
  size_t elems() const { return (size_t)n * hp() * wp() * c; }
  int cf() const { return ta_fmt_is_half(fmt) ? c / 2 : c; }
  size_t off(int img, int y, int x) const { return (((size_t)img * hp() + y + halo) * wp() + x + halo) * cf(); }
};

struct ta_strides {
  int img, row, pix, off0;
};
static inline ta_strides ta_tensor_strides(const ta_tensor& t, int pad, bool count_c) {
  const int s = count_c ? t.c : t.cf(), sh = t.halo - pad;
  return {(int)((size_t)t.hp() * t.wp() * s), t.wp() * s, s, (int)(((size_t)sh * t.wp() + sh) * s)};
}

struct ta_conv_launch {
  const float* in;
  const float* w;
  const int32_t* ktab;
  const float* bias;
  const float* prelu;
  float* out;
  const float* res;
  float* out2;
  const float* scale2;
  const float* shift2;
  int M, Ho, Wo, n_slabs, coutp, cout, act, stride, prec;
  int uniform_k, k_cblocks, k_w, k_h, in_ch_off;
  int in_img, in_row, in_pix, in_off0;
  int out_img, out_row, out_pix, out_off0, out_ch, out_fmt;
  int res_img, res_row, res_pix, res_off0, res_up2, res_ch, res_fmt;
  int o2_img, o2_row, o2_pix, o2_off0, o2_ch, o2_fmt;
  int in_fmt;
  int win_wp, win_img;
  int group_cout, group_cin;
  int k_split;
  float* partial;
  int variant;
  const float* dw_w;
  const float* dw_bias;
  int dw_c, dw_stride;
  int pool;
  float r_nct, r_tile_blocks, r_Wo, r_Ho, r_HoWo;
  int fast_div;
  int fast_drain;
#ifdef TA_CONV_TRACE
  int trace_block;
#endif
  const float* bias9;
  int range_check;
  int amax_index;
  int* range_flag;
};

static inline int ta_split_fmt_of(int prec) { return prec == 0 ? 0  : (prec == 4 ? 3  : ((prec == 3 || prec == 5) ? 2  : 1 )); }

static inline int ta_conv_ksplit(int coutp, int n_slabs, bool eligible, int packed = 0) {
  if (!eligible || coutp % 128) return 1;
  if (packed > 1) return packed <= n_slabs ? packed : 1;
  if (n_slabs < 512) return 1;
  return 32;
}

struct ta_k_geometry {
  int kblk;
  bool uniform;
  int cblocks;
};
static inline ta_k_geometry ta_conv_k_geometry(const ta_op_desc& op, int in_fmt) {
  const int kblk = ta_fmt_is_half(in_fmt) ? 64 : 32;
  return {kblk, op.cin % kblk == 0 && op.n_slabs == (int64_t)op.kh * op.kw * (op.cin / kblk), op.cin / kblk};
}
static inline int ta_op_ksplit(const ta_op_desc& op, int in_fmt) {
  const bool eligible = ta_conv_k_geometry(op, in_fmt).uniform && in_fmt == ta_split_fmt_of(op.prec) && op.groups <= 1 && !op.pool;
  return ta_conv_ksplit(op.coutp, op.n_slabs, eligible, ta_op_packed_ksplit(op));
}

int ta_launch_conv(ta_ctx* ctx, const ta_conv_launch& p, double flops);
int ta_launch_conv_sym(ta_ctx* ctx, int variant, const ta_conv_launch& p);
int ta_launch_conv_split(ta_ctx* ctx, int variant, const ta_conv_launch& p);
int ta_launch_conv_split_modes(ta_ctx* ctx, int variant, const ta_conv_launch& p);
int ta_launch_dwpw(ta_ctx* ctx, const ta_conv_launch& p, double flops);
int ta_win_patch_rows(const ta_conv_launch& p, int BM);
#define TA_WIN_PR_2x2 384
#define TA_WIN_PR_2x4 448
#define TA_WIN_PR_1x4 512
struct ta_frames;
int ta_launch_rfstem(ta_ctx* ctx, const uint8_t* frames_dev, int n, int h, int w, const float* weights_host, const float* w2_dev, const struct ta_tensor& out);

struct ta_dw_launch {
  const float* in;
  const float* w;
  const float* bias;
  float* out;
  int N, Ho, Wo, C, stride, relu;
  int in_img, in_row, in_pix, in_off0, in_fmt;
  int out_img, out_row, out_pix, out_off0, out_fmt;
};
int ta_launch_dwconv(ta_ctx* ctx, const ta_dw_launch& p);
int ta_launch_maxpool(ta_ctx* ctx, const ta_tensor& in, const ta_tensor& out, int n);
int ta_launch_copych(ta_ctx* ctx, const ta_tensor& in, int in_ch, const ta_tensor& out, int out_ch, int ch, int n);

enum { TA_PRE_RETINAFACE = 1, TA_PRE_OPENPOSE = 2, TA_PRE_ARCFACE_CROPS = 3 };
int ta_launch_preprocess(ta_ctx* ctx, int mode, const uint8_t* src_dev, int n, int h, int w, const ta_tensor& dst);

struct ta_plan {
  int n = 0, h = 0, w = 0;
  std::vector<ta_tensor> tensors;
  char* arena = nullptr;
  size_t arena_bytes = 0;
  int32_t* ktab_dev = nullptr;
  std::vector<size_t> ktab_off;
  float* splitk_ws = nullptr;
  uint64_t last_use = 0;
  ta_plan() = default;
  ta_plan(const ta_plan&) = delete;
  ~ta_plan() {
    if (arena) (void)hipFree(arena);
    if (ktab_dev) (void)hipFree(ktab_dev);
  }
};

struct ta_program {
  ta_blob_header hdr;
  std::vector<ta_tensor_desc> tdesc;
  std::vector<ta_op_desc> ops;
};
int ta_program_parse(int kind, const void* blob, size_t bytes, ta_program* out, char* msg, size_t msg_capacity);

struct ta_model : ta_program {
  ta_ctx* ctx = nullptr;
  int kind = 0;
  char* weights_dev = nullptr;
  bool has_half_ops = false;
  bool amax_on = false;
  std::vector<char> tensor_read;
  std::vector<std::vector<float>> unscale_host;
  std::vector<char> weights_host_small;
  std::vector<std::unique_ptr<ta_plan>> plans;
  ta_plan* active = nullptr;
  uint64_t use_counter = 0;
  int run_n = 0;
  const uint8_t* input_u8 = nullptr;
  const ta_tensor& tensor(int i) const { return active->tensors[i]; }
  ~ta_model() {
    plans.clear();
    if (weights_dev) (void)hipFree(weights_dev);
  }
};

int ta_model_plan(ta_model* m, int n, int h, int w);
int ta_model_run_ops(ta_model* m);
```

### terran_amd/lib.py

```python
import ctypes as C
import os

import numpy as np

HERE = os.path.dirname(os.path.abspath(__file__))
LIB_PATH = os.path.join(HERE, 'libterran_amd.so')

OK, E_INVALID, E_DEVICE, E_CAPACITY, E_OVERFLOW, E_RANGE = 0, -1, -2, -3, -4, -5
_CODES = {E_INVALID: 'TA_E_INVALID', E_DEVICE: 'TA_E_DEVICE', E_CAPACITY: 'TA_E_CAPACITY', E_OVERFLOW: 'TA_E_OVERFLOW',
          E_RANGE: 'TA_E_RANGE'}


class TerranAmdError(RuntimeError):
    def __init__(self, code, msg):
        super().__init__('%s: %s' % (_CODES.get(code, code), msg))
        self.code = code


c_int, c_float, c_double, c_void_p, c_size_t = C.c_int, C.c_float, C.c_double, C.c_void_p, C.c_size_t
P = C.POINTER
u8p, i32p, f32p, f64p = P(C.c_uint8), P(C.c_int32), P(C.c_float), P(C.c_double)

SIGNATURES = {
    'ta_version': (C.c_char_p, []),
# ... 13 lines not shown
    'ta_frames_upload': (c_int, [c_void_p, c_void_p, c_int, c_int, c_int, P(c_void_p)]),
    'ta_frames_alloc': (c_int, [c_void_p, c_int, c_int, c_int, P(c_void_p)]),
    'ta_frames_shape': (c_int, [c_void_p, P(c_int), P(c_int), P(c_int)]),
    'ta_frames_download': (c_int, [c_void_p, c_void_p]),
    'ta_frames_free': (None, [c_void_p]),
    'ta_frames_resize': (c_int, [c_void_p, c_void_p, c_int, c_int, P(c_void_p)]),
    'ta_frames_resize_bicubic': (c_int, [c_void_p, c_void_p, c_int, c_int, P(c_void_p)]),
    'ta_frames_paste': (c_int, [c_void_p, c_void_p, c_int, c_void_p, c_int, c_int, c_int]),
    'ta_frames_draw': (c_int, [c_void_p, c_void_p, c_void_p, c_int]),
    'ta_frames_draw_masks': (c_int, [c_void_p, c_void_p, c_void_p, c_int, c_void_p, c_size_t]),
    'ta_frames_blur': (c_int, [c_void_p, c_void_p, c_void_p, c_int]),
    'ta_blur_plan': (c_int, [c_void_p, c_int, c_void_p, c_void_p, c_void_p]),
    'ta_frames_resample': (c_int, [c_void_p, c_void_p, c_void_p, c_int, c_int, c_int, c_int, P(c_void_p)]),
    'ta_resample_plan': (c_int, [c_int, c_double, c_double, c_int, c_int, c_void_p, c_void_p, c_int, P(c_int)]),
    'ta_frames_pixelate': (c_int, [c_void_p, c_void_p, c_void_p, c_int]),
    'ta_frames_transform': (c_int, [c_void_p, c_void_p, c_void_p, c_int, c_int, c_int, c_int, c_void_p, P(c_void_p)]),
    'ta_frames_transform_mesh': (c_int, [c_void_p, c_void_p, c_void_p, c_int, c_void_p, c_int, c_void_p, c_int, c_int, c_int, c_int,
                                         c_void_p, P(c_void_p)]),
    'ta_mesh_plan': (c_int, [c_void_p, c_int, c_int, c_int, c_void_p, c_void_p, c_void_p, c_void_p, c_int, P(c_int)]),
    'ta_frames_transpose': (c_int, [c_void_p, c_void_p, c_int, P(c_void_p)]),
    'ta_frames_histogram': (c_int, [c_void_p, c_void_p, c_void_p, c_int, c_int, c_void_p]),
    'ta_frames_point': (c_int, [c_void_p, c_void_p, c_void_p, c_int, c_void_p, c_int]),
    'ta_frames_saturate': (c_int, [c_void_p, c_void_p, c_void_p, c_int]),
    'ta_frames_filter': (c_int, [c_void_p, c_void_p, c_void_p, c_int, c_void_p, c_int]),
    'ta_filter_plan': (c_int, [c_void_p, c_int, c_void_p, c_int, c_void_p, c_void_p, c_void_p]),
    'ta_frames_color': (c_int, [c_void_p, c_void_p, c_void_p, c_int, c_void_p, c_int, c_void_p, c_size_t]),
    'ta_color_plan': (c_int, [c_void_p, c_int, c_void_p, c_int, c_void_p, c_size_t, c_void_p, c_void_p]),
    'ta_yuv_frame_bytes': (c_size_t, [c_int, c_int, c_int]),
    'ta_frames_from_yuv': (c_int, [c_void_p, c_void_p, c_int, c_int, c_int, c_void_p, P(c_void_p)]),
    'ta_frames_to_yuv': (c_int, [c_void_p, c_void_p, c_void_p, c_void_p]),
    'ta_yuv_convert_samples': (c_int, [c_void_p, c_int, c_void_p, c_size_t, c_void_p]),
    'ta_frames_combine': (c_int, [c_void_p, c_void_p, c_void_p, c_void_p, c_void_p, c_int, c_void_p, c_size_t]),
    'ta_jpeg_coefficients': (c_int, [c_void_p, c_size_t, c_void_p, c_void_p, C.c_int64, C.c_char_p, c_int]),
    'ta_jpeg_decode': (c_int, [c_void_p, P(c_void_p), P(c_size_t), c_int, c_int, c_int, P(c_void_p), P(C.c_int32),
                               P(C.c_int32)]),
    'ta_jpeg_last_stats': (c_int, [c_void_p, c_void_p, c_void_p]),
    'ta_jpeg_encode_header': (c_int, [c_int, c_int, c_int, c_int, c_void_p, c_size_t, P(c_size_t)]),
    'ta_jpeg_encode': (c_int, [c_void_p, c_void_p, c_int, c_int, P(c_void_p), P(c_size_t)]),
    'ta_jpeg_encode_last_stats': (c_int, [c_void_p, c_void_p, c_void_p]),
    'ta_jpeg_encode_opt': (c_int, [c_void_p, c_void_p, c_int, c_int, c_int, P(c_void_p), P(c_size_t)]),
    'ta_jpeg_optimal_table': (c_int, [c_void_p, c_void_p, c_void_p, P(c_int)]),
    'ta_jpeg_encode_last_opt_stats': (c_int, [c_void_p, c_void_p]),
    'ta_program_check': (c_int, [c_int, c_void_p, c_size_t, C.c_char_p, c_size_t]),
    'ta_model_load': (c_int, [c_void_p, c_int, c_void_p, c_size_t, P(c_void_p)]),
    'ta_model_free': (None, [c_void_p]),
    'ta_model_kind': (c_int, [c_void_p]),
    'ta_model_forward_frames': (c_int, [c_void_p, c_void_p]),
    'ta_model_forward_crops': (c_int, [c_void_p, c_void_p, c_int]),
    'ta_model_tensor_shape': (c_int, [c_void_p, c_int, P(c_int), P(c_int), P(c_int), P(c_int)]),
    'ta_model_tensor_unscale': (c_int, [c_void_p, c_int, c_void_p, c_int]),
    'ta_model_debug_amax': (c_int, [c_void_p, c_int, c_void_p, c_int]),
    'ta_model_graph_probe': (c_int, [c_void_p, c_int, c_void_p]),
    'ta_model_read_tensor': (c_int, [c_void_p, c_int, c_int, c_int, c_void_p]),
    'ta_retinaface_run': (c_int, [c_void_p, c_void_p, c_float, c_float, c_int, c_void_p, c_void_p, c_void_p,
                                  c_void_p, P(C.c_int32)]),
    'ta_retinaface_postprocess': (c_int, [c_void_p, P(c_void_p), c_int, c_int, c_int, c_float, c_float, c_int,
                                          c_void_p, c_void_p, c_void_p, c_void_p, P(C.c_int32)]),
    'ta_arcface_embed_crops': (c_int, [c_void_p, c_void_p, c_int, c_int, c_void_p]),
    'ta_arcface_embed_faces': (c_int, [c_void_p, c_void_p, c_void_p, c_void_p, c_int, c_int, c_void_p, c_void_p]),
    'ta_arcface_embed_faces_multi': (c_int, [c_void_p, P(c_void_p), c_int, c_void_p, c_void_p, c_void_p, c_int, c_int, c_void_p,
                                             c_void_p]),
    'ta_cosine_distance': (c_int, [c_void_p, c_void_p, c_int, c_void_p, c_int, c_int, c_void_p]),
    'ta_gallery_create': (c_int, [c_void_p, c_int, C.c_int64, P(c_void_p)]),
    'ta_gallery_free': (None, [c_void_p]),
    'ta_gallery_add': (c_int, [c_void_p, c_void_p, c_void_p, C.c_int64, c_int]),
    'ta_gallery_remove': (c_int, [c_void_p, c_void_p, c_int, P(C.c_int64)]),
    'ta_gallery_clear': (c_int, [c_void_p]),
    'ta_gallery_size': (c_int, [c_void_p, P(C.c_int64), P(C.c_int64)]),
    'ta_gallery_download': (c_int, [c_void_p, c_void_p, c_void_p]),
    'ta_gallery_search': (c_int, [c_void_p, c_void_p, c_int, c_int, c_int, c_void_p, c_void_p, c_void_p]),
    'ta_gallery_cluster': (c_int, [c_void_p, C.c_float, c_int, c_void_p, c_void_p, P(C.c_int32), P(C.c_int32)]),
    'ta_openpose_run': (c_int, [c_void_p, c_void_p, c_double, c_int, c_void_p, c_void_p, c_void_p, P(C.c_int32)]),
    'ta_openpose_group': (c_int, [c_void_p, c_void_p, c_void_p, c_int, c_int, c_int, c_double, c_int, c_void_p,
                                  c_void_p, c_void_p, P(C.c_int32)]),
    'ta_bicubic_x8': (c_int, [c_void_p, c_void_p, c_int, c_int, c_int, c_int, c_void_p]),
    'ta_openpose_last_stats': (c_int, [c_void_p, c_void_p, c_void_p]),
    'ta_openpose_debug_read': (c_int, [c_void_p, c_int, c_int, c_void_p, c_void_p, c_void_p, c_int, c_void_p, c_void_p,
                                       c_void_p]),
    'ta_openpose_debug_capacity': (c_int, [c_void_p, c_int, c_void_p]),
    'ta_debug_conv_variant': (c_int, [c_void_p, c_int]),
    'ta_debug_range_check': (c_int, [c_void_p]),
    'ta_debug_conv_counts': (c_int, [c_void_p, c_void_p, c_int]),
    'ta_debug_kernel_work': (c_int, [c_void_p, C.c_char_p, c_size_t, c_int]),
}

GALLERY_ROW_TILE, GALLERY_QUERY_GROUP, GALLERY_MAX_K = 128, 32, 16
GALLERY_CLUSTER_MAX_ROWS = 1 << 18

DRAW_BAR, DRAW_LINE, DRAW_DISC, DRAW_MASK = 0, 1, 2, 3
PRIM_DT = np.dtype([('frame', '<i4'), ('kind', '<i4'), ('x0', '<i4'), ('y0', '<i4'), ('x1', '<i4'), ('y1', '<i4'),
                    ('width', '<i4'), ('rgba', 'u1', (4,))])
assert PRIM_DT.itemsize == 32

BLUR_BOX, BLUR_ELLIPSE = 0, 1
BLUR_DT = np.dtype([('frame', '<i4'), ('x0', '<i4'), ('y0', '<i4'), ('x1', '<i4'), ('y1', '<i4'), ('shape', '<i4'),
                    ('radius', '<f4')])
assert BLUR_DT.itemsize == 28


def blur_plan(regions):
    lib = load()
    regions, p, n = _records(regions, BLUR_DT)
    rounds, fr, w = np.zeros(n, np.int32), np.zeros(n, np.float32), np.zeros((n, 2), np.uint32)
    rc = lib.ta_blur_plan(p, n, ptr(rounds), ptr(fr), ptr(w))
    if rc != OK:
        raise TerranAmdError(rc, 'blur_plan: an empty or inverted box, an unknown shape or a bad radius')
    return rounds, fr, w


NEAREST, LANCZOS, BILINEAR, BICUBIC, BOX, HAMMING = 0, 1, 2, 3, 4, 5
RESAMPLE_FILTERS = {'nearest': NEAREST, 'lanczos': LANCZOS, 'bilinear': BILINEAR, 'bicubic': BICUBIC, 'box': BOX,
                    'hamming': HAMMING}
RESAMPLE_DT = np.dtype([('frame', '<i4'), ('x0', '<f4'), ('y0', '<f4'), ('x1', '<f4'), ('y1', '<f4')])
assert RESAMPLE_DT.itemsize == 20
PIXELATE_DT = np.dtype([('frame', '<i4'), ('x0', '<i4'), ('y0', '<i4'), ('x1', '<i4'), ('y1', '<i4'), ('shape', '<i4'),
                        ('block', '<i4')])
assert PIXELATE_DT.itemsize == 28
RESAMPLE_SIDE_LIMIT = 16384

HIST_RGB, HIST_L = 0, 1
HIST_MODES = {'RGB': HIST_RGB, 'L': HIST_L}
HIST_DT = np.dtype([('frame', '<i4'), ('x0', '<i4'), ('y0', '<i4'), ('x1', '<i4'), ('y1', '<i4'), ('shape', '<i4')])
assert HIST_DT.itemsize == 24
POINT_DT = np.dtype([('frame', '<i4'), ('x0', '<i4'), ('y0', '<i4'), ('x1', '<i4'), ('y1', '<i4'), ('shape', '<i4'),
                     ('lut', '<i4')])
assert POINT_DT.itemsize == 28
SATURATE_DT = np.dtype([('frame', '<i4'), ('x0', '<i4'), ('y0', '<i4'), ('x1', '<i4'), ('y1', '<i4'), ('shape', '<i4'),
                        ('factor', '<f4')])
assert SATURATE_DT.itemsize == 28

FILTER_KERNEL, FILTER_RANK, FILTER_UNSHARP = 0, 1, 2
FILTER_REGION_DT = np.dtype([('frame', '<i4'), ('x0', '<i4'), ('y0', '<i4'), ('x1', '<i4'), ('y1', '<i4'), ('shape', '<i4'),
                             ('spec', '<i4')])
assert FILTER_REGION_DT.itemsize == 28
FILTER_SPEC_DT = np.dtype([('kind', '<i4'), ('size', '<i4'), ('rank', '<i4'), ('has_factor', '<i4'), ('kernel', '<f4', (25,)),
                           ('scale', '<f4'), ('offset', '<f4'), ('factor', '<f4'), ('radius', '<f4'), ('percent', '<i4'),
                           ('threshold', '<i4')])
assert FILTER_SPEC_DT.itemsize == 140

(COMBINE_PASTE, COMBINE_BLEND, COMBINE_LIGHTER, COMBINE_DARKER, COMBINE_DIFFERENCE, COMBINE_MULTIPLY, COMBINE_SCREEN, COMBINE_ADD,
 COMBINE_SUBTRACT, COMBINE_ADD_MODULO, COMBINE_SUBTRACT_MODULO, COMBINE_SOFT_LIGHT, COMBINE_HARD_LIGHT, COMBINE_OVERLAY) = range(14)
COMBINE_OPS = {'paste': COMBINE_PASTE, 'blend': COMBINE_BLEND, 'lighter': COMBINE_LIGHTER, 'darker': COMBINE_DARKER,
               'difference': COMBINE_DIFFERENCE, 'multiply': COMBINE_MULTIPLY, 'screen': COMBINE_SCREEN, 'add': COMBINE_ADD,
               'subtract': COMBINE_SUBTRACT, 'add_modulo': COMBINE_ADD_MODULO, 'subtract_modulo': COMBINE_SUBTRACT_MODULO,
               'soft_light': COMBINE_SOFT_LIGHT, 'hard_light': COMBINE_HARD_LIGHT, 'overlay': COMBINE_OVERLAY}
MASK_NONE, MASK_CONSTANT, MASK_BITMAP, MASK_FRAMES = 0, 1, 2, 3
COMBINE_DT = np.dtype([('frame', '<i4'), ('x0', '<i4'), ('y0', '<i4'), ('x1', '<i4'), ('y1', '<i4'), ('shape', '<i4'),
                       ('src_frame', '<i4'), ('src_x', '<i4'), ('src_y', '<i4'), ('op', '<i4'), ('alpha', '<f4'), ('offset', '<i4'),
                       ('mask_kind', '<i4'), ('mask_value', '<i4'), ('mask_frame', '<i4'), ('mask_x', '<i4'), ('mask_y', '<i4'),
                       ('mask_band', '<i4')])
assert COMBINE_DT.itemsize == 72

COLOR_MATRIX, COLOR_RGB2YCBCR, COLOR_YCBCR2RGB, COLOR_RGB2HSV, COLOR_HSV2RGB, COLOR_LUT3D = range(6)
COLOR_REGION_DT = np.dtype([('frame', '<i4'), ('x0', '<i4'), ('y0', '<i4'), ('x1', '<i4'), ('y1', '<i4'), ('shape', '<i4'),
                            ('op', '<i4')])
assert COLOR_REGION_DT.itemsize == 28
COLOR_OP_DT = np.dtype([('kind', '<i4'), ('size', '<i4', (3,)), ('table', '<i4')])
assert COLOR_OP_DT.itemsize == 20


def _color_args(ops, tables):
    ops = np.ascontiguousarray(ops, dtype=COLOR_OP_DT).reshape(-1)
    tables = np.ascontiguousarray(tables if tables is not None else [], dtype=np.float32).reshape(-1)
    return ops, tables


# ... 111 lines not shown
    rc = lib.ta_mesh_plan(p, n, out_h, out_w, None, None, None, None, -1, C.byref(k))
    if rc != E_CAPACITY:
        raise TerranAmdError(rc, 'mesh_plan: a bad output size, box or corner, or more cells or tile entries than the limits')
    tiles = -(-out_w // MESH_TILE_W) * -(-out_h // MESH_TILE_H)
    coefs, boxes = np.zeros((n, 8), np.float64), np.zeros((n, 4), np.int32)
    first, entries = np.zeros(tiles + 1, np.int32), np.zeros(k.value, np.int32)
    rc = lib.ta_mesh_plan(p, n, out_h, out_w, ptr(coefs), ptr(boxes), ptr(first), ptr(entries), k.value, C.byref(k))
    if rc != OK:
        raise TerranAmdError(rc, 'mesh_plan')
    return coefs, boxes, first, entries


def transpose_op(op):
    if isinstance(op, str) and op.lower() in TRANSPOSE_OPS:
        return TRANSPOSE_OPS[op.lower()]
    if isinstance(op, (int, np.integer)) and not isinstance(op, bool) and 0 <= int(op) <= 6:
        return int(op)
    raise ValueError('op must be one of %s or Pillow\'s code 0 .. 6, got %r' % (sorted(TRANSPOSE_OPS), op))


JPEG_DEVICE = 0
JPEG_INVALID = -1
JPEG_PATHS = {-1: 'invalid', 0: 'device', 1: 'progressive/lossless/hierarchical', 2: 'arithmetic', 3: 'precision',
              4: 'components', 5: 'rgb', 6: 'scans', 7: 'sampling'}
JPEG_HEADER_DT = np.dtype([('width', '<i4'), ('height', '<i4'), ('components', '<i4'), ('path', '<i4'),
                           ('h_samp', '<i4', (3,)), ('v_samp', '<i4', (3,)), ('quant_index', '<i4', (3,)),
                           ('blocks_w', '<i4', (3,)), ('blocks_h', '<i4', (3,)), ('restart_interval', '<i4'),
                           ('reserved', '<i4', (2,)), ('block_offset', '<i8', (3,)), ('blocks_total', '<i8'),
                           ('quant', '<u2', (4, 64))])
assert JPEG_HEADER_DT.itemsize == 632


def jpeg_coefficients(data, header_only=False):
    lib = load()
    buf = np.frombuffer(bytes(data), np.uint8)
    hdr = np.zeros(1, JPEG_HEADER_DT)
    err = C.create_string_buffer(256)
    rc = lib.ta_jpeg_coefficients(ptr(buf), buf.size, ptr(hdr), None, 0, err, len(err))
    if rc != OK:
        raise TerranAmdError(rc, err.value.decode(errors='replace'))
    if header_only or hdr['path'][0] != JPEG_DEVICE:
        return hdr[0], None
    coefs = np.empty((int(hdr['blocks_total'][0]), 64), np.int16)
    rc = lib.ta_jpeg_coefficients(ptr(buf), buf.size, ptr(hdr), ptr(coefs), coefs.shape[0], err, len(err))
    if rc != OK:
        raise TerranAmdError(rc, err.value.decode(errors='replace'))
    return hdr[0], coefs


def jpeg_encode_header(h, w, quality=75, subsampling=2):
    lib = load()
    size = c_size_t()
    buf = np.zeros(1024, np.uint8)
    rc = lib.ta_jpeg_encode_header(int(h), int(w), int(quality), int(subsampling), ptr(buf), buf.size, C.byref(size))
    if rc != OK:
        raise TerranAmdError(rc, 'jpeg_encode_header(%r, %r, %r, %r)' % (h, w, quality, subsampling))
    return buf[:size.value].tobytes()


def jpeg_optimal_table(freq):
    lib = load()
    f = np.zeros(257, np.int64)
    freq = np.asarray(freq, np.int64).reshape(-1)
    f[:min(256, freq.size)] = freq[:256]
    bits, vals, n = np.zeros(17, np.uint8), np.zeros(256, np.uint8), c_int()
    rc = lib.ta_jpeg_optimal_table(ptr(f), ptr(bits), ptr(vals), C.byref(n))
    if rc != OK:
        raise TerranAmdError(rc, 'jpeg_optimal_table: frequencies must be 0 .. 10^9 - 1 and not all zero')
    return bits[1:].tolist(), vals[:n.value].tolist()


def check_program(program_or_blob, kind=None):
    lib = load()
    if isinstance(program_or_blob, (bytes, bytearray, memoryview)):
        blob = bytes(program_or_blob)
        if kind is None:
            raise ValueError('check_program: the bytes of a blob need `kind` (a pack.MODEL_* constant)')
    else:
        blob, kind = program_or_blob.blob(), program_or_blob.kind if kind is None else kind
    err = C.create_string_buffer(256)
    rc = lib.ta_program_check(int(kind), blob, len(blob), err, len(err))
    if rc != OK:
        raise TerranAmdError(rc, err.value.decode(errors='replace'))


def check_jpeg_options(quality, subsampling):
    if isinstance(quality, bool) or not isinstance(quality, (int, np.integer)) or not 1 <= quality <= 100:
        raise ValueError('JPEG quality must be an int in 1..100, got %r' % (quality,))
    if isinstance(subsampling, bool) or not isinstance(subsampling, (int, np.integer)) or subsampling not in (0, 1, 2):
        raise ValueError('JPEG subsampling must be 0 (4:4:4), 1 (4:2:2) or 2 (4:2:0), got %r' % (subsampling,))
    return int(quality), int(subsampling)


def check_jpeg_optimize(optimize):
    if not isinstance(optimize, (bool, np.bool_)):
        raise ValueError('JPEG optimize must be True or False, got %r' % (optimize,))
    return bool(optimize)


CONV_VARIANTS = {'auto': 0, 'generic': 1, 'pipe64': 2, 'pipe128': 3, 'split_2x2': 4, 'split_2x2_p8': 5, 'split_2x4': 6,
                 'split_1x4': 7, 'win_2x2': 8, 'win_2x4': 9, 'win_1x4': 10, 'split_1x4_w2': 11, 'split_2x2_w2': 12}

_lib = None


def load():
    global _lib
    if _lib is None:
        if not os.path.exists(LIB_PATH):
            raise TerranAmdError(E_DEVICE, 'libterran_amd.so not built (run `python -m terran_amd.build`); '
                                           'there is no CPU fallback')
        from . import build as _build
        try:
            with open(_build.STAMP) as fh:
                stamp = fh.read().strip()
        except OSError:
            stamp = None
        try:
            current = _build.source_hash()
        except OSError:
            current = stamp
        if (stamp is None or stamp != current) and not os.environ.get('TA_ALLOW_STALE_LIB'):
            raise TerranAmdError(E_DEVICE, 'libterran_amd.so was not built from the sources in terran_amd/csrc '
                                           '(run `python -m terran_amd.build`)')
        os.environ.setdefault('GPU_MAX_HW_QUEUES', '12')
        os.environ.setdefault('HIP_FORCE_DEV_KERNARG', '1')
        lib = C.CDLL(LIB_PATH)
        missing = []
        for name, (res, args) in SIGNATURES.items():
            try:
                fn = getattr(lib, name)
            except AttributeError:
                missing.append(name)
                continue
            fn.restype = res
            fn.argtypes = args
        if missing and not os.environ.get('TA_BRINGUP_ALLOW_MISSING'):
            raise TerranAmdError(E_INVALID, 'libterran_amd.so lacks ABI symbols: %s' % ', '.join(missing))
        _lib = lib
    return _lib


def ptr(a):
    return a.ctypes.data_as(c_void_p) if a is not None else None


def _records(a, dtype):
    a = np.ascontiguousarray(a, dtype=dtype)
    return a, (ptr(a) if len(a) else None), len(a)


class Context:

    def __init__(self, device_id=0):
        self.lib = load()
        h = c_void_p()
        rc = self.lib.ta_ctx_create(int(device_id), C.byref(h))
        if rc != OK:
            raise TerranAmdError(rc, 'ta_ctx_create(%d) failed: no usable gfx950 device '
                                     '(ta_device_count=%d)' % (device_id, self.lib.ta_device_count()))
        self.h = h
        self.device_id = device_id

    def check(self, rc):
        if rc != OK:
            raise TerranAmdError(rc, self.lib.ta_last_error(self.h).decode(errors='replace'))
# ... 49 lines not shown
        if per and n > 0 and data.size != n * per:
            raise ValueError('frames_from_yuv: %d bytes are not %d frames of %d bytes' % (data.size, n, per))
        hd = c_void_p()
        self.check(self.lib.ta_frames_from_yuv(self.h, ptr(data), n, h, w, ptr(s), C.byref(hd)))
        return Frames(self, handle=hd)

    def pinned_array(self, shape):
        n = int(np.prod(shape))
        p = c_void_p()
        self.check(self.lib.ta_host_alloc(self.h, n, C.byref(p)))
        arr = np.ctypeslib.as_array((C.c_uint8 * n).from_address(p.value)).reshape(shape)
        arr_ptr = p.value
        return arr, arr_ptr

    def free_pinned(self, ptr):
        if getattr(self, 'h', None):
            self.lib.ta_host_free(self.h, c_void_p(ptr))

    def cosine_distance(self, a, b):
        a = np.ascontiguousarray(a, dtype=np.float32)
        b = np.ascontiguousarray(b, dtype=np.float32)
        out = np.empty((a.shape[0], b.shape[0]), np.float32)
        self.check(self.lib.ta_cosine_distance(self.h, ptr(a), a.shape[0], ptr(b), b.shape[0], a.shape[1], ptr(out)))
        return out

    def jpeg_decode(self, buffers, threads=0):
        bufs = [bytes(b) for b in buffers]
        n = len(bufs)
        arrs = [np.frombuffer(b, np.uint8) for b in bufs]
        data = (c_void_p * n)(*[a.ctypes.data for a in arrs])
        sizes = (c_size_t * n)(*[a.size for a in arrs])
        out = (c_void_p * n)()
        paths = np.zeros(n, np.int32)
        req = C.c_int32()
        rc = self.lib.ta_jpeg_decode(self.h, data, sizes, n, int(threads), n, out, paths.ctypes.data_as(P(C.c_int32)),
                                     C.byref(req))
        if rc != OK:
            e = TerranAmdError(rc, self.last_error())
            e.paths = paths
            raise e
        return [Frames(self, handle=c_void_p(out[k])) for k in range(req.value)], paths

    def jpeg_stats(self):
        ms, cnt = np.zeros(4, np.float64), np.zeros(4, np.int64)
        self.check(self.lib.ta_jpeg_last_stats(self.h, ptr(ms), ptr(cnt)))
        return (dict(zip(('host', 'h2d', 'idct', 'color'), ms.tolist())),
                dict(zip(('images', 'blocks', 'bytes', 'fallbacks'), cnt.tolist())))

    def jpeg_encode(self, frames, quality=75, subsampling=2, optimize=False):
        quality, subsampling = check_jpeg_options(quality, subsampling)
        optimize = check_jpeg_optimize(optimize)
        n = frames.shape[0]
        out = c_void_p()
        sizes = (c_size_t * n)()
        if optimize:
            self.check(self.lib.ta_jpeg_encode_opt(self.h, frames.h, quality, subsampling, 1, C.byref(out), sizes))
        else:
            self.check(self.lib.ta_jpeg_encode(self.h, frames.h, quality, subsampling, C.byref(out), sizes))
        files, at = [], out.value
        for k in range(n):
            files.append(C.string_at(at, sizes[k]))
            at += sizes[k]
        return files

    def jpeg_encode_stats(self):
        ms, cnt, opt = np.zeros(8, np.float64), np.zeros(4, np.int64), np.zeros(2, np.float64)
        self.check(self.lib.ta_jpeg_encode_last_stats(self.h, ptr(ms), ptr(cnt)))
        self.check(self.lib.ta_jpeg_encode_last_opt_stats(self.h, ptr(opt)))
        return (dict(zip(('h2d', 'coef', 'length', 'emit', 'ffcount', 'pack', 'd2h', 'host', 'statistics', 'tables'),
                         ms.tolist() + opt.tolist())),
                dict(zip(('images', 'blocks', 'bytes', 'entropy_bytes'), cnt.tolist())))

    def conv_variant(self, name):
        self.check(self.lib.ta_debug_conv_variant(self.h, CONV_VARIANTS[name]))

    def conv_counts(self, reset=False):
        c = np.zeros(16, np.int64)
        self.check(self.lib.ta_debug_conv_counts(self.h, ptr(c), int(reset)))
        out = {k: int(c[v]) for k, v in CONV_VARIANTS.items() if v and c[v]}
        if c[15]:
            out['lean_epilogue'] = int(c[15])
        return out

    def kernel_work(self, reset=False):
        buf = C.create_string_buffer(1 << 16)
        self.check(self.lib.ta_debug_kernel_work(self.h, buf, len(buf), int(reset)))
        out = {}
        for line in buf.value.decode().splitlines():
            f = line.split(';')
            out[f[0]] = (int(f[1]), float(f[2]), float(f[3]) if len(f) > 3 else 0.0)
        return out

    def pose_debug(self, n, cap_peaks=1024, cap_conn=1024):
        pc = np.zeros((n, 18), np.int32)
        pyx = np.zeros((n, 18, cap_peaks, 2), np.int32)
        psc = np.zeros((n, 18, cap_peaks), np.float32)
        cc = np.zeros((n, 19), np.int32)
        cij = np.zeros((n, 19, cap_conn, 2), np.int32)
        csc = np.zeros((n, 19, cap_conn), np.float32)
        self.check(self.lib.ta_openpose_debug_read(self.h, n, cap_peaks, ptr(pc), ptr(pyx), ptr(psc), cap_conn,
                                                   ptr(cc), ptr(cij), ptr(csc)))
        assert pc.max(initial=0) <= cap_peaks and cc.max(initial=0) <= cap_conn
        peaks = [[(pyx[i, p, :pc[i, p]].copy(), psc[i, p, :pc[i, p]].copy()) for p in range(18)] for i in range(n)]
        conns = [[None if cc[i, l] < 0 else (cij[i, l, :cc[i, l]].copy(), csc[i, l, :cc[i, l]].copy())
                  for l in range(19)] for i in range(n)]
        return peaks, conns

    def pose_debug_capacity(self, n):
        cap = np.zeros(n, np.int32)
        self.check(self.lib.ta_openpose_debug_capacity(self.h, n, ptr(cap)))
        return cap.tolist()

    def pose_stats(self):
        a, b = C.c_int64(), C.c_int64()
        self.check(self.lib.ta_openpose_last_stats(self.h, C.byref(a), C.byref(b)))
        return a.value, b.value

    def bicubic_x8(self, maps):
        maps = np.ascontiguousarray(maps, dtype=np.float32)
        n, c, h, w = maps.shape
        out = np.empty((n, c, 8 * h, 8 * w), np.float32)
        self.check(self.lib.ta_bicubic_x8(self.h, ptr(maps), n, c, h, w, ptr(out)))
        return out


class Frames:

    def __init__(self, ctx, images=None, handle=None):
        self.ctx = ctx
        if handle is not None:
            self.h = handle
        else:
            h = c_void_p()
            n, hh, ww = images.shape[:3]
            ctx.check(ctx.lib.ta_frames_upload(ctx.h, ptr(images), n, hh, ww, C.byref(h)))
            self.h = h
        n, hh, ww = c_int(), c_int(), c_int()
        ctx.lib.ta_frames_shape(self.h, C.byref(n), C.byref(hh), C.byref(ww))
        self.shape = (n.value, hh.value, ww.value, 3)

    def __len__(self):
        return self.shape[0]

    @classmethod
    def zeros(cls, ctx, n, h, w):
        hd = c_void_p()
        ctx.check(ctx.lib.ta_frames_alloc(ctx.h, n, h, w, C.byref(hd)))
        return cls(ctx, handle=hd)

    def resize(self, h, w, ctx=None):
        ctx = ctx or self.ctx
        hd = c_void_p()
        ctx.check(ctx.lib.ta_frames_resize(ctx.h, self.h, int(h), int(w), C.byref(hd)))
        return Frames(ctx, handle=hd)

    def resize_bicubic(self, h, w, ctx=None):
        ctx = ctx or self.ctx
        hd = c_void_p()
        ctx.check(ctx.lib.ta_frames_resize_bicubic(ctx.h, self.h, int(h), int(w), C.byref(hd)))
        return Frames(ctx, handle=hd)

    def paste(self, src, src_index, dst_index, top, left):
        self.ctx.check(self.ctx.lib.ta_frames_paste(self.ctx.h, src.h, src_index, self.h, dst_index, top, left))

    def draw(self, prims, masks=None, ctx=None):
        ctx = ctx or self.ctx
# ... 261 lines not shown
```

### terran_amd/pack/__init__.py

```python
from .arcface import pack_arcface
from .layout import (ACT_NONE, ACT_PRELU, ACT_RELU, BLOB_VERSION, FMT_F16, FMT_F32, FMT_SPLIT, FMT_SPLIT16, HEADER_DT, MAGIC,
                     MODEL_ARCFACE, MODEL_OPENPOSE, MODEL_RETINAFACE, OP_CONV, OP_COPYCH, OP_DT, OP_DWCONV, OP_DWPW, OP_MAXPOOL,
                     OP_RFSTEM, PRECISIONS, SPLIT_FMT, TENSOR_DT, fold_input_affine, row_exponents, split_bf16_rows, split_f16_rows)
from .moments import _ACT_TARGET_LOG2, _CH_SPREAD, act_moments
from .openpose import pack_openpose
from .program import Program
from .retinaface import pack_retinaface
from .switches import PACK_SWITCHES, active_switches, source_tag

PACKERS = {MODEL_RETINAFACE: pack_retinaface, MODEL_ARCFACE: pack_arcface, MODEL_OPENPOSE: pack_openpose}
```

### terran_amd/pack/layout.py

```python
import numpy as np

MODEL_RETINAFACE, MODEL_ARCFACE, MODEL_OPENPOSE = 1, 2, 3
OP_CONV, OP_DWCONV, OP_MAXPOOL, OP_COPYCH, OP_RFSTEM, OP_DWPW = 1, 2, 3, 4, 5, 6
ACT_NONE, ACT_RELU, ACT_PRELU = 0, 1, 2
MAGIC = 0x314D4154

HEADER_DT = np.dtype({
    'names': ['magic', 'version', 'kind', 'n_tensors', 'n_ops', 'input_tensor', 'n_outputs', 'outputs',
              'tensors_off', 'ops_off', 'weights_off', 'weights_bytes'],
    'formats': ['<u4', '<u4', '<i4', '<i4', '<i4', '<i4', '<i4', ('<i4', 16), '<i8', '<i8', '<i8', '<i8'],
    'offsets': [0, 4, 8, 12, 16, 20, 24, 28, 96, 104, 112, 120],
    'itemsize': 128,
})
TENSOR_DT = np.dtype([('channels', '<i4'), ('halo', '<i4'), ('alias_of', '<i4'), ('fmt', '<i4'), ('unscale_off', '<i4')])
FMT_F32, FMT_SPLIT, FMT_SPLIT16, FMT_F16 = 0, 1, 2, 3
_OP_I32 = ['type', 'in', 'out', 'in_ch_off', 'cin', 'out_ch_off', 'cout', 'coutp', 'kh', 'kw', 'stride', 'pad',
           'act', 'res', 'res_ch_off', 'res_up2', 'out2', 'out2_ch_off', 'n_slabs', 'prec', 'groups', 'variant', 'pool', 'wscale_log2']
_OP_I64 = ['w_off', 'bias_off', 'prelu_off', 'scale2_off', 'shift2_off', 'wus_off']
OP_DT = np.dtype([(n, '<i4') for n in _OP_I32] + [(n, '<i8') for n in _OP_I64] + [('macs_per_pixel', '<f8')])
assert OP_DT.itemsize == 152 and TENSOR_DT.itemsize == 20
BLOB_VERSION = 9

PRECISIONS = {'f32': 0, 'bf16x3': 1, 'bf16': 2, 'f16x3': 3, 'f16': 4, 'f16x2': 5}
SPLIT_FMT = {0: FMT_F32, 1: FMT_SPLIT, 2: FMT_SPLIT, 3: FMT_SPLIT16, 4: FMT_F16, 5: FMT_SPLIT16}

_OP_DEFAULTS = dict(in_ch_off=0, out_ch_off=0, coutp=0, kh=1, kw=1, stride=1, pad=0, act=ACT_NONE, res=-1, res_ch_off=0, res_up2=0,
                    out2=-1, out2_ch_off=0, n_slabs=0, prec=0, groups=1, variant=0, pool=0, wscale_log2=0,
                    w_off=-1, bias_off=-1, prelu_off=-1, scale2_off=-1, shift2_off=-1, wus_off=-1, macs_per_pixel=0.0)


def op_desc(typ, tin, tout, cin, cout, **fields):
    op = dict(_OP_DEFAULTS, type=typ, out=tout, cin=cin, cout=cout, **fields)
    op['in'] = tin
    assert set(op) == set(OP_DT.names), set(op) ^ set(OP_DT.names)
    return op


def _rup(x, m):
    return (x + m - 1) // m * m


class WeightRegion:

    def __init__(self):
        self.chunks = []
        self.nbytes = 0
        self._at = {}

    def reserve(self, nbytes, data=None):
        off, nbytes = self.nbytes, int(nbytes)
        self._at[off] = (len(self.chunks), nbytes)
        self.chunks.append(data)
        pad = -nbytes % 256
        if pad:
            self.chunks.append(b'\0' * pad)
        self.nbytes += nbytes + pad
        return off

    def add(self, arr):
        data = np.ascontiguousarray(arr, dtype=np.float32).tobytes()
        return self.reserve(len(data), data)

    def rewrite(self, off, data):
        if not isinstance(data, bytes):
            data = np.ascontiguousarray(data, dtype=np.float32).tobytes()
        k, size = self._at[off]
        assert len(data) == size, (len(data), size)
        self.chunks[k] = data

    def tobytes(self):
        return b''.join(self.chunks)


def _bf16_bits(x):
    u = np.ascontiguousarray(x, dtype=np.float32).view(np.uint32)
    return ((u + np.uint32(0x7FFF) + ((u >> np.uint32(16)) & np.uint32(1))) >> np.uint32(16)).astype(np.uint16)


def _bf16_to_f32(b):
    return (b.astype(np.uint32) << np.uint32(16)).view(np.float32)


def split_bf16_rows(packed):
    hi = _bf16_bits(packed)
    lo = _bf16_bits(packed - _bf16_to_f32(hi))
    rows = np.concatenate([hi, lo], axis=-1)
    return np.ascontiguousarray(rows).view(np.float32)


def row_exponents(packed):
    m = np.abs(np.asarray(packed, np.float32)).max(axis=(0, 2)).astype(np.float64)
    ok = np.isfinite(m) & (m > 0)
    s = np.zeros(m.shape, np.int64)
    s[ok] = np.clip(13 - np.floor(np.log2(m[ok])), -60, 60).astype(np.int64)
    return s


def split_f16_rows(packed, exps=None):
# ... 28 lines not shown
```

### terran_amd/pack/openpose.py

```python
import numpy as np

from .. import arch
from .layout import ACT_NONE, ACT_RELU, MODEL_OPENPOSE, OP_COPYCH, OP_MAXPOOL
from .program import Program

OP_FEAT, OP_PAF, OP_HM, OP_XCH = 0, 128, 168, 192


def pack_openpose(sd, precision='f32'):
    if precision in ('f16', 'f16x2'):
        precision = 'f16x3'
    P = Program(MODEL_OPENPOSE, precision)
    t = P.tensor(4, 1, name='input')
    P.input_tensor = t
    P.input_stats = (np.array([-0.05, -0.05, -0.05, 0.0]), np.array([0.08, 0.08, 0.08, 0.0]))
    X0 = P.tensor(OP_XCH, 3, name='X0')
    X1 = P.tensor(OP_XCH, 3, name='X1')
    items = arch.OPENPOSE_MODEL0
    skip_pool = False
    for i, item in enumerate(items):
        nxt = items[i + 1] if i + 1 < len(items) else None
        if item[0] == 'pool':
            if skip_pool:
                skip_pool = False
                continue
            o = P.tensor(P.tensors[t][0], 1)
            P.simple(OP_MAXPOOL, t, o)
            t = o
            continue
        name, cin, cout, k = item
        W, b = sd['model0.%s.weight' % name], sd['model0.%s.bias' % name]
        if nxt is None:
            P.conv(t, X0, W, b, act=ACT_RELU, out_ch_off=OP_FEAT)
            P.tap('feat', X0, OP_FEAT, 128)
        elif nxt[0] == 'pool' and cin % 32 == 0 and cout % 64 == 0:
            o = P.tensor(cout, 1, name=name + '_pooled')
            P.conv(t, o, W, b, act=ACT_RELU, pool=True)
            t = o
            skip_pool = True
        else:
            o = P.tensor(cout, 0 if nxt[0] == 'pool' else 1, name=name)
            P.conv(t, o, W, b, act=ACT_RELU)
            t = o
    P.simple(OP_COPYCH, X0, X1, OP_FEAT, OP_FEAT, 128)

    cat_pos = np.concatenate([OP_PAF + np.arange(38), OP_HM + np.arange(19), OP_FEAT + np.arange(128)])
    for st in range(1, 7):
        xin, xout = (X0, X1) if st % 2 == 1 else (X1, X0)
        l1, l2 = arch.openpose_stage_layers(st, 1), arch.openpose_stage_layers(st, 2)
        (n1, cin, c1, k, r1), (n2, cin2, c2, k2, r2) = l1[0], l2[0]
        assert (cin, k, r1) == (cin2, k2, r2) and c1 == c2 == 128
        W = np.concatenate([np.asarray(sd['model%d_%d.%s.weight' % (st, br, n)]) for br, n in ((1, n1), (2, n2))])
        b = np.concatenate([np.asarray(sd['model%d_%d.%s.bias' % (st, br, n)]) for br, n in ((1, n1), (2, n2))])
        kw = dict(ch_pos=cat_pos, cin_p=OP_XCH) if cin == 185 else dict(in_ch_off=OP_FEAT)
        cur = P.tensor(c1 + c2, l1[1][3] // 2)
        P.conv(xin, cur, W, b, act=ACT_RELU if r1 else ACT_NONE, **kw)
        for li in range(1, len(l1) - 1):
            (na, cin, cout, k, relu), (nb, cin2, cout2, k2, relu2) = l1[li], l2[li]
            assert (cin, cout, k, relu) == (cin2, cout2, k2, relu2) and cin % 32 == 0 and cout % 128 == 0
            W = np.concatenate([np.asarray(sd['model%d_%d.%s.weight' % (st, br, n)]) for br, n in ((1, na), (2, nb))])
            b = np.concatenate([np.asarray(sd['model%d_%d.%s.bias' % (st, br, n)]) for br, n in ((1, na), (2, nb))])
            o = P.tensor(2 * cout, l1[li + 1][3] // 2)
            P.conv(cur, o, W, b, act=ACT_RELU if relu else ACT_NONE, groups=2)
            cur = o
        (np_, cin, co1, k, r1), (nh, cin2, co2, k2, r2) = l1[-1], l2[-1]
        if r1 == r2 and cin == cin2 <= 128:
            Wp, bp = np.asarray(sd['model%d_1.%s.weight' % (st, np_)]), np.asarray(sd['model%d_1.%s.bias' % (st, np_)])
            Wh, bh = np.asarray(sd['model%d_2.%s.weight' % (st, nh)]), np.asarray(sd['model%d_2.%s.bias' % (st, nh)])
            Wm = np.zeros((60, 2 * cin, 1, 1), np.float32)
            bm = np.zeros(60, np.float32)
            Wm[0:co1, :cin], bm[0:co1] = Wp, bp
            Wm[40:40 + co2, cin:], bm[40:40 + co2] = Wh, bh
            P.conv(cur, xout, Wm, bm, act=ACT_RELU if r1 else ACT_NONE, out_ch_off=OP_PAF, cout_p=60)
            P.ops[-1]['macs_per_pixel'] = float((co1 + co2) * cin)
        else:
            for br, layers in ((1, l1), (2, l2)):
                name, cin, cout, k, relu = layers[-1]
                key = 'model%d_%d.%s' % (st, br, name)
                off, cp = (OP_PAF, 40) if br == 1 else (OP_HM, 20)
                P.conv(cur, xout, sd[key + '.weight'], sd[key + '.bias'], act=ACT_RELU if relu else ACT_NONE,
                       in_ch_off=(br - 1) * cin, out_ch_off=off, cout_p=cp)
        P.tap('stage%d_paf' % st, xout, OP_PAF, 38)
        P.tap('stage%d_hm' % st, xout, OP_HM, 19)
    P.outputs = [X0]
    P.tap('pafs', X0, OP_PAF, 38)
    P.tap('heatmaps', X0, OP_HM, 19)
    return P
```

### terran_amd/pack/program.py

```python
import json
import os

import numpy as np

from . import moments, storage
from .layout import (ACT_NONE, ACT_RELU, BLOB_VERSION, FMT_F16, HEADER_DT, MAGIC, OP_CONV, OP_DT, OP_DWCONV, OP_DWPW, OP_MAXPOOL,
                     OP_RFSTEM, PRECISIONS, TENSOR_DT, WeightRegion, _rup, fold_input_affine, op_desc, pack_rows)
from .moments import ChannelStats, act_bound, act_moments


def _pow2(e):
    return np.ldexp(1.0, np.asarray(e).astype(np.int32))


class Program:

    def __init__(self, kind, precision='f32'):
        self.kind = kind
        self.precision = precision
        self.prec = PRECISIONS[precision]
        self.tensors = []
        self.ops = []
        self.w = WeightRegion()
        self.names = {}
        self.extra = {}
        self.input_tensor = None
        self.outputs = []
        self.f32_only = set()
        self.allow_split = True
        self.lane = 0
        self.stats = {}
        self._fold = {}
        self.input_stats = None
        self.forced_scale = {}
        self.scales_enabled = not os.environ.get('TERRAN_AMD_NO_ACT_SCALES')

    def tensor(self, channels, halo, alias_of=-1, name=None, f32=False):
        assert channels % 4 == 0
        self.tensors.append((channels, halo, alias_of))
        tid = len(self.tensors) - 1
        if f32:
            self.f32_only.add(tid)
        if name:
            self.names[name] = (tid, 0, channels)
        return tid

    def tap(self, name, tid, ch_off, ch):
        self.names[name] = (tid, ch_off, ch)

    def _stats_of(self, tid):
        c, _, a = self.tensors[tid]
        if a >= 0:
            st = self._stats_of(a)
            return st.tiled(c // len(st.mean))
        if tid not in self.stats:
            mu, var = np.zeros(c), np.ones(c)
            if tid == self.input_tensor and self.input_stats is not None:
                m_, v_ = self.input_stats
                mu[:len(m_)], var[:len(v_)] = m_, v_
            self.stats[tid] = ChannelStats.unwritten(mu, var)
            if tid == self.input_tensor:
                self.stats[tid].written[:] = True
        return self.stats[tid]

    def _emit(self, op, fold=None):
        if fold is not None:
            self._fold[len(self.ops)] = fold
        self.ops.append(op)

    def conv(self, tin, tout, W, bias, *, stride=1, pad=None, act=ACT_NONE, in_ch_off=0, ch_pos=None, cin_p=None,
             out_ch_off=0, cout_p=None, prelu=None, res=-1, res_ch_off=0, res_up2=0, out2=-1, out2_ch_off=0,
             scale2=None, shift2=None, groups=1, variant=0, pool=False, k_split=0, precision=None, in_affine=None):
        W = np.asarray(W, dtype=np.float64)
        cout, cin, kh, kw = W.shape
        bias9 = None
        if in_affine is not None:
            assert (kh, kw, stride) == (3, 3, 1) and pad in (None, 1) and groups == 1 and out2 < 0 and scale2 is None and not pool
            W, bias9 = fold_input_affine(W, bias, *in_affine)
            bias = bias9[5]
        if groups > 1:
            assert cout % groups == 0 and cin % 32 == 0 and (cout // groups) % 128 == 0 and ch_pos is None
        if pad is None:
            pad = kh // 2
        if pool:
            assert groups == 1 and res < 0 and out2 < 0 and stride == 1 and cin % 32 == 0 and cout % 64 == 0 and ch_pos is None
        if cin_p is None:
            cin_p = _rup(cin, 4)
        if ch_pos is None:
            ch_pos = np.arange(cin)
        if cout_p is None:
            cout_p = _rup(cout, 4)
        coutp = _rup(cout_p, 32)
        K = kh * kw * cin_p
        n_slabs = _rup(K, 32) // 32
        full = np.zeros((kh * kw, cin_p, coutp), np.float32)
        full[:, np.asarray(ch_pos), :cout] = W.transpose(2, 3, 1, 0).reshape(kh * kw, cin, cout)
        flat = np.zeros((n_slabs * 32, coutp), np.float32)
        flat[:K] = full.reshape(K, coutp)
        prec = self.prec if precision is None else PRECISIONS[precision]

        def vec(v, fill=0.0):
            if v is None:
                return -1, None
            out = np.full(coutp, fill, np.float64)
            out[:cout] = np.asarray(v, dtype=np.float64)
            return self.w.add(out), out
        fold = dict(flat=flat, taps=kh * kw, cin_p=cin_p, K=K)
        if bias9 is not None:
            t9 = np.zeros((16, coutp), np.float64)
            t9[:, :cout] = bias9
            scale2_off = self.w.add(t9)
            fold['bias9'] = t9
            variant |= 1 << 16
        else:
            scale2_off, fold['scale2'] = vec(scale2)
        bvec = np.zeros(coutp, np.float64)
        if bias is not None:
            bvec[:cout] = np.asarray(bias, np.float64)
        fold['bias'] = bvec
        bias_off = self.w.add(np.concatenate([bvec, np.ones(coutp)]))
        prelu_off, _ = vec(prelu)
        shift2_off, fold['shift2'] = vec(shift2)
        self._emit(op_desc(OP_CONV, tin, tout, cin_p, cout_p, in_ch_off=in_ch_off, out_ch_off=out_ch_off, coutp=coutp, kh=kh, kw=kw,
                           stride=stride, pad=pad, act=act, res=res, res_ch_off=res_ch_off, res_up2=res_up2, out2=out2,
                           out2_ch_off=out2_ch_off, n_slabs=n_slabs, prec=prec, groups=groups,
                           variant=variant | (int(k_split) << 8) | (self.lane << 17), pool=int(bool(pool)),
                           w_off=self.w.reserve(n_slabs * coutp * 128), bias_off=bias_off, prelu_off=prelu_off,
                           scale2_off=scale2_off, shift2_off=shift2_off, wus_off=bias_off + 4 * coutp,
# ... 68 lines not shown
                           wus_off=bias_off + 4 * coutp, macs_per_pixel=float(cout * C)),
                   dict(flat=flat, bias=bias, dw_w=w9, dw_b=bd, mid_bound=mid_bound))
        mu2, var2 = moments.pointwise_moments(Wp.reshape(cout, C), bias[:cout], *act_moments(mu0, var0, ACT_RELU))
        self._stats_of(tout).write(0, *act_moments(mu2, var2, ACT_RELU), act_bound(mu2, var2, ACT_RELU))

    def simple(self, typ, tin, tout, in_ch_off=0, out_ch_off=0, ch=0):
        self._emit(op_desc(typ, tin, tout, ch, ch, in_ch_off=in_ch_off, out_ch_off=out_ch_off, kh=2, kw=2, stride=2))
        st = self._stats_of(tin)
        if typ == OP_MAXPOOL:
            self._stats_of(tout).write(0, *moments.pool_moments(st.mean, st.var), st.amax.copy())
        else:
            sl = slice(in_ch_off, in_ch_off + ch)
            self._stats_of(tout).write(out_ch_off, st.mean[sl].copy(), st.var[sl].copy(), st.amax[sl].copy())

    @classmethod
    def from_cache(cls, path):
        with open(path, 'rb') as f:
            head = f.read(16)
            if head[:8] != b'TAMCACHE':
                raise ValueError('not a pack cache file')
            n = int.from_bytes(head[8:16], 'little')
            meta = json.loads(f.read(n).decode())
            blob = f.read()
        self = cls(meta['kind'], meta['precision'])
        self.names = {k: tuple(v) for k, v in meta['names'].items()}
        self.outputs = meta['outputs']
        self.extra = dict(meta.get('extra') or {})
        self._blob = blob
        return self

    def save_cache(self, path):
        meta = json.dumps({'kind': self.kind, 'precision': self.precision, 'names': self.names,
                           'outputs': [int(o) for o in self.outputs], 'extra': getattr(self, 'extra', {})}).encode()
        tmp = path + '.tmp.%d' % os.getpid()
        with open(tmp, 'wb') as f:
            f.write(b'TAMCACHE' + len(meta).to_bytes(8, 'little') + meta + self.blob())
        os.replace(tmp, path)

    def tensor_formats(self):
        return storage.tensor_formats(self)

    def expected_amax(self, tid, per_channel=False):
        st = self._stats_of(tid)
        am = np.where(st.written, st.amax, 0.0)
        return am if per_channel else float(am.max()) if len(am) else 0.0

    def tensor_scales(self):
        return storage.tensor_scales(self)

    def blob(self):
        if getattr(self, '_blob', None) is not None:
            return self._blob
        fmts = self.tensor_formats()
        self.scales = scales = self.tensor_scales()
        tens = self._tensor_table(fmts, scales)
        self.mid_scales = {}
        finish = {OP_CONV: self._finish_conv, OP_DWPW: self._finish_dwpw, OP_RFSTEM: self._finish_rfstem}
        for i, f in self._fold.items():
            op = self.ops[i]
            finish[op['type']](i, op, f, scales[op['in']], self._exponents(scales, op, 'out'), fmts)
        ops = np.zeros(len(self.ops), OP_DT)
        for i, op in enumerate(self.ops):
            for k, v in op.items():
                ops[i][k] = v
        t_off = HEADER_DT.itemsize
        o_off = t_off + tens.nbytes
        w_off = _rup(o_off + ops.nbytes, 256)
        outs = np.full(16, -1, np.int32)
        outs[:len(self.outputs)] = self.outputs
        hdr = np.zeros(1, HEADER_DT)
        hdr[0] = (MAGIC, BLOB_VERSION, self.kind, len(self.tensors), len(self.ops), self.input_tensor, len(self.outputs), outs,
                  t_off, o_off, w_off, self.w.nbytes)
        head = hdr.tobytes() + tens.tobytes() + ops.tobytes()
        for f in self._fold.values():
            f.pop('flat', None)
        self._blob = head + b'\0' * (w_off - len(head)) + self.w.tobytes()
        return self._blob

    def _tensor_table(self, fmts, scales):
        tens = np.zeros(len(self.tensors), TENSOR_DT)
        for i, (c, h, a) in enumerate(self.tensors):
            unscale_off = self.w.add(_pow2(-scales[i])) if np.any(scales[i] != 0) else -1
            assert unscale_off < 2 ** 31
            tens[i] = (c, h, a, fmts[i], unscale_off)
        return tens

    @staticmethod
    def _exponents(scales, op, which):
        a = np.zeros(op['coutp'], np.int64)
        off = op[which + '_ch_off']
        seg = scales[op[which]][off:off + op['cout']]
        a[:len(seg)] = seg
        return a

    def _rewrite_bias(self, op, f, a_out, wexp):
        self.w.rewrite(op['bias_off'], np.concatenate([f['bias'] * _pow2(a_out), _pow2(a_out - wexp)]))

    @staticmethod
    def _fold_input_exponents(op, f, a_in):
        flat, taps, cin_p, K = f['flat'], f['taps'], f['cin_p'], f['K']
        groups = max(op['groups'], 1)
        cols = a_in[op['in_ch_off']:op['in_ch_off'] + cin_p * groups]
        if not np.any(cols != 0):
            return flat
        fs = flat.copy()
        cg = op['cout'] // groups if groups > 1 else flat.shape[1]
        for g in range(groups):
            e = -np.tile(cols[g * cin_p:(g + 1) * cin_p], taps).astype(np.int32)
            fs[:K, g * cg:(g + 1) * cg] = np.ldexp(flat[:K, g * cg:(g + 1) * cg], e[:, None])
        return fs

    def _finish_conv(self, i, op, f, a_in, a_out, fmts):
        fs = self._fold_input_exponents(op, f, a_in)
        data, wexp = pack_rows(fs, op['coutp'], op['prec'])
        if op['prec'] == 4 and fmts[op['in']] == FMT_F16:
            cin_p, K, coutp = f['cin_p'], f['K'], op['coutp']
            assert cin_p % 64 == 0 and op['in_ch_off'] == 0 and op['groups'] == 1
            rows = np.ldexp(fs[:K].reshape(K // 64, 64, coutp).transpose(0, 2, 1), wexp[None, :, None].astype(np.int32)).astype(np.float16)
            assert rows.nbytes * 2 == len(data)
            data = rows.tobytes() + b'\0' * rows.nbytes
            op['n_slabs'] = K // 64
            f['rows64'] = rows
        f['wexp'] = wexp
        self.w.rewrite(op['w_off'], data)
        self._rewrite_bias(op, f, a_out, wexp)
        if 'bias9' in f:
            self.w.rewrite(op['scale2_off'], f['bias9'] * _pow2(a_out)[None, :])
        elif op['out2'] >= 0:
            a2 = self._exponents(self.scales, op, 'out2')
            self.w.rewrite(op['scale2_off'], f['scale2'] * _pow2(a2 - a_out))
            self.w.rewrite(op['shift2_off'], f['shift2'] * _pow2(a2))

    def _finish_dwpw(self, i, op, f, a_in, a_out, fmts):
        C = op['cin']
        a_mid = np.zeros(C, np.int64)
        if op['prec'] == 3 and self.scales_enabled:
            mb = f['mid_bound']
            okc = np.isfinite(mb) & (mb > 0)
            if okc.any():
                a_mid[okc] = moments.scale_exponents(np.maximum(mb, moments.spread_floor(mb[okc].max()))[okc])
        elif op['prec'] == 0:
            a_mid = a_in[:C].copy()
        if ('mid', i) in self.forced_scale:
            a_mid[:] = int(self.forced_scale[('mid', i)])
        self.mid_scales[i] = a_mid
        self.w.rewrite(op['scale2_off'], f['dw_w'] * _pow2(a_mid - a_in[:C])[None, :])
        self.w.rewrite(op['shift2_off'], f['dw_b'] * _pow2(a_mid))
        fl = f['flat'].copy()
        fl[:C] = np.ldexp(fl[:C], -a_mid.astype(np.int32)[:, None])
        data, wexp = pack_rows(fl, op['coutp'], op['prec'])
        self.w.rewrite(op['w_off'], data)
        self._rewrite_bias(op, f, a_out, wexp)

    def _finish_rfstem(self, i, op, f, a_in, a_out, fmts):
        parts, up = list(f['rfstem']), _pow2(a_out)
        if len(parts) == 10:
            parts[8] = (parts[8].reshape(16, 32) * up[None, :32]).ravel()
            parts[9] = parts[9] * up[:32]
        else:
            parts[4] = (parts[4].reshape(16, 8) * up[:16, None]).ravel()
            parts[5] = parts[5] * up[:16]
        self.w.rewrite(op['w_off'], np.concatenate(parts))
```

Measured before the change: 2268 frames/s.

## Add batch-innermost layout for OpenPose 7x7 convs and skip padded taps

Introduces a batch-innermost tensor layout (images interleaved per pixel) for the OpenPose refinement-stage 7x7 conv chain. The split conv kernel now computes per-tile kernel-tap masks from the spatial extent of the output tile and skips K slabs whose taps land entirely in zero padding. With the batch folded into the width dimension, each tile covers few spatial columns, so more border taps can be skipped. Adds loader validation, 4 GiB extent checks and debug counters. Risks include changed memory access strides for these convs and extra per-block mask setup.

```diff
diff --git a/include/terran_amd.h b/include/terran_amd.h
--- a/include/terran_amd.h
+++ b/include/terran_amd.h
@@ -366,6 +366,8 @@
 int ta_debug_conv_variant(ta_ctx* ctx, int variant);
 int ta_debug_range_check(ta_ctx* ctx);
 int ta_debug_conv_counts(ta_ctx* ctx, int64_t* counts16, int reset);
+int ta_debug_conv_slabs(ta_ctx* ctx, int64_t* out2, int enable, int reset);
+int ta_debug_tap_masks(int images, int h, int w, int n, int pad, int kh, int kw, int pt0, int bm, unsigned* masks2);
 int ta_debug_kernel_work(ta_ctx* ctx, char* csv, size_t capacity, int reset);
 
 #ifdef __cplusplus
diff --git a/terran_amd/csrc/conv_common.h b/terran_amd/csrc/conv_common.h
--- a/terran_amd/csrc/conv_common.h
+++ b/terran_amd/csrc/conv_common.h
@@ -1,5 +1,7 @@
 #pragma once
 #include <stdio.h>
+
+#include <algorithm>
 
 #include "act_format.h"
 #include "ta_internal.h"
@@ -221,7 +223,7 @@
     cblocks = p.k_cblocks;
     kw = p.k_w;
     kh = p.k_h;
-    pix_bytes = p.in_pix * 4;
+    pix_bytes = p.tap_pix * 4;
     row_bytes = p.in_row * 4;
     if (s0 == 0) {
       cb = kx = ky = b_off = a_slab = 0;
@@ -250,7 +252,35 @@
       }
     }
   }
+  __device__ __forceinline__ bool kept(unsigned kym, unsigned kxm) const { return ((kym >> ky) & (kxm >> kx) & 1u) != 0; }
+  __device__ __forceinline__ void seek_kept(unsigned kym, unsigned kxm) {
+    while (!kept(kym, kxm) && cb < cblocks) advance();
+  }
+  __device__ __forceinline__ void advance_kept(unsigned kym, unsigned kxm) {
+    do advance();
+    while (!kept(kym, kxm) && cb < cblocks);
+  }
 };
+
+__host__ __device__ inline unsigned ta_tap_span(int lo, int hi, int size, int pad, int k) {
+  int a = pad - hi, b = size - 1 + pad - lo;
+  if (a < 0) a = 0;
+  if (b > k - 1) b = k - 1;
+  if (b < a) return 0u;
+  return (b - a + 1 >= 32 ? ~0u : ((1u << (b - a + 1)) - 1u)) << a;
+}
+__host__ __device__ inline void ta_tap_masks(int img0, int y0, int c0, int img1, int y1, int c1, int H, int W, int pad, int kh, int kw,
+                                             unsigned& kym, unsigned& kxm) {
+  const bool same_img = img0 == img1;
+  const bool next_img = img1 == img0 + 1;
+  if (same_img) kym = ta_tap_span(y0, y1, H, pad, kh);
+  else if (next_img && y1 < y0) kym = ta_tap_span(y0, H - 1, H, pad, kh) | ta_tap_span(0, y1, H, pad, kh);
+  else kym = ta_tap_span(0, H - 1, H, pad, kh);
+  const bool next_row = (same_img && y1 == y0 + 1) || (next_img && y0 == H - 1 && y1 == 0);
+  if (same_img && y0 == y1) kxm = ta_tap_span(c0, c1, W, pad, kw);
+  else if (next_row && c1 < c0) kxm = ta_tap_span(c0, W - 1, W, pad, kw) | ta_tap_span(0, c1, W, pad, kw);
+  else kxm = ta_tap_span(0, W - 1, W, pad, kw);
+}
 
 __device__ __forceinline__ int ta_div_r(int t, int d, float rd, int fast) {
   if (!fast) return t / d;
@@ -804,6 +834,27 @@
   ta_tile_grid(const ta_conv_launch& p, int BN, int BM) : n_ct(p.coutp / BN), n_pt((p.M + BM - 1) / BM), groups(((n_pt + 7) / 8) * n_ct) {}
 };
 
+static inline int ta_tap_tile_kept(const ta_conv_launch& q, int pt0, int BM, unsigned* kym_out = nullptr, unsigned* kxm_out = nullptr) {
+  const int last = pt0 + (q.M - pt0 < BM ? q.M - pt0 : BM) - 1, HoWo = q.Ho * q.Wo;
+  unsigned kym = q.k_h >= 32 ? ~0u : (1u << q.k_h) - 1u, kxm = q.k_w >= 32 ? ~0u : (1u << q.k_w) - 1u;
+  if (q.skip_n > 0) {
+    unsigned my, mx;
+    ta_tap_masks(pt0 / HoWo, pt0 % HoWo / q.Wo, pt0 % q.Wo / q.skip_n, last / HoWo, last % HoWo / q.Wo, last % q.Wo / q.skip_n, q.skip_h, q.skip_w,
+                 q.skip_pad, q.k_h, q.k_w, my, mx);
+    if (my && mx) kym = my, kxm = mx;
+  }
+  if (kym_out) *kym_out = kym;
+  if (kxm_out) *kxm_out = kxm;
+  return __builtin_popcount(kym) * __builtin_popcount(kxm);
+}
+static inline int64_t ta_tap_tile_slabs(const ta_conv_launch& q, int BM) {
+  const int n_pt = (q.M + BM - 1) / BM;
+  if (q.skip_n <= 0) return (int64_t)n_pt * q.n_slabs;
+  int64_t total = 0;
+  for (int t = 0; t < n_pt; ++t) total += (int64_t)ta_tap_tile_kept(q, t * BM, BM) * q.k_cblocks;
+  return total;
+}
+
 #define TA_NOTE_KERNEL(ctx, ...)                                    \
   do {                                                              \
     static char _name[80];                                          \
diff --git a/terran_amd/csrc/conv_igemm.hip b/terran_amd/csrc/conv_igemm.hip
--- a/terran_amd/csrc/conv_igemm.hip
+++ b/terran_amd/csrc/conv_igemm.hip
@@ -10,6 +10,7 @@
   const bool split_in = p.in_fmt == ta_split_fmt_of(p.prec);
   const bool deep = p.uniform_k && (p.n_slabs >= 2 || p.prec == PREC_F16);
   const bool staged = ((p.out_ch | p.res_ch | p.o2_ch) & 7) == 0 && (p.cout & 3) == 0;
+  if ((p.tap_pix != p.in_pix || p.in_base0) && !is_split_variant(v)) return false;
   switch (v) {
     case TA_CV_GENERIC: return p.in_fmt == TA_FMT_F32 && !p.group_cout;
     case TA_CV_PIPE64: return deep && staged && p.coutp % 64 == 0 && !p.group_cout && (p.in_fmt == TA_FMT_F32 || (split_in && p.prec != PREC_F16));
@@ -87,6 +88,7 @@
   p.trace_block = ctx->conv_trace_block;
 #endif
   if (p.k_split < 1 || !p.partial) p.k_split = 1;
+  if (!p.tap_pix) p.tap_pix = p.in_pix;
   if (p.coutp % 32 != 0 || p.cout % 4 != 0) return ta_fail(ctx, TA_E_INVALID, "conv: bad cout padding");
   if (p.prec != PREC_F32 && p.prec != PREC_BF16X3 && p.prec != PREC_BF16 && p.prec != PREC_F16X3 && p.prec != PREC_F16 && p.prec != PREC_F16X2)
     return ta_fail(ctx, TA_E_INVALID, "conv: unknown precision mode %d", p.prec);
@@ -144,6 +146,40 @@
   return TA_OK;
 }
 
+int ta_debug_conv_slabs(ta_ctx* ctx, int64_t* out2, int enable, int reset) {
+  if (!ctx) return TA_E_INVALID;
+  if (out2) {
+    out2[0] = ctx->slabs_full;
+    out2[1] = ctx->slabs_run;
+  }
+  if (reset) ctx->slabs_full = ctx->slabs_run = 0;
+  if (enable >= 0) ctx->slab_counting = enable != 0;
+  return TA_OK;
+}
+
+int ta_debug_tap_masks(int images, int h, int w, int n, int pad, int kh, int kw, int pt0, int bm, unsigned* masks2) {
+  if (images < 1 || h < 1 || w < 1 || n < 1 || pad < 0 || kh < 1 || kw < 1 || kh > 32 || kw > 32 || bm < 1 || pt0 < 0) return TA_E_INVALID;
+  ta_conv_launch q;
+  memset(&q, 0, sizeof(q));
+  q.Ho = h;
+  q.Wo = w * n;
+  q.M = images * h * w * n;
+  if (pt0 >= q.M) return TA_E_INVALID;
+  q.k_h = kh;
+  q.k_w = kw;
+  q.skip_n = n;
+  q.skip_h = h;
+  q.skip_w = w;
+  q.skip_pad = pad;
+  unsigned kym, kxm;
+  const int kept = ta_tap_tile_kept(q, pt0, bm, &kym, &kxm);
+  if (masks2) {
+    masks2[0] = kym;
+    masks2[1] = kxm;
+  }
+  return kept;
+}
+
 int ta_debug_conv_counts(ta_ctx* ctx, int64_t* counts16, int reset) {
   if (!ctx) return TA_E_INVALID;
   for (int i = 0; i < TA_CV_COUNT; ++i) {
diff --git a/terran_amd/csrc/conv_split_kernels.h b/terran_amd/csrc/conv_split_kernels.h
--- a/terran_amd/csrc/conv_split_kernels.h
+++ b/terran_amd/csrc/conv_split_kernels.h
@@ -83,6 +83,23 @@
     s_begin = (int)(((long long)ks * p.n_slabs) / p.k_split);
     S = (int)(((long long)(ks + 1) * p.n_slabs) / p.k_split) - s_begin;
   }
+  unsigned kym = ~0u, kxm = ~0u;
+  if (p.skip_n) {
+    const ta_pixel_walk tw(p, pt0, HoWo);
+    int img1, y1, x1;
+    tw.at((p.M - pt0 < BM ? p.M - pt0 : BM) - 1, img1, y1, x1);
+    const int c0 = ta_div_r(tw.x0, p.skip_n, p.skip_rn, 1), c1 = ta_div_r(x1, p.skip_n, p.skip_rn, 1);
+    unsigned my, mx;
+    ta_tap_masks(tw.img0, tw.y0, c0, img1, y1, c1, p.skip_h, p.skip_w, p.skip_pad, p.k_h, p.k_w, my, mx);
+    my = __builtin_amdgcn_readfirstlane(my);
+    mx = __builtin_amdgcn_readfirstlane(mx);
+    const int kept = __builtin_popcount(my) * __builtin_popcount(mx);
+    if (kept) {
+      kym = my;
+      kxm = mx;
+      S = kept * p.k_cblocks;
+    }
+  }
 
   if (wave >= NC) {
     const int pw = wave - NC;
@@ -95,20 +112,23 @@
 #pragma unroll
     for (int q = 0; q < QA; ++q) a_off[q] = (unsigned)(((ct0 + (q * NP + pw) * 8 + (lane >> 3)) * 32 + lchunk * 4) * 4);
     ta_k_walk wa(p, s_begin);
+    wa.seek_kept(kym, kxm);
     auto issue_a = [&](int, int stage) {
 #pragma unroll
       for (int q = 0; q < QA; ++q) ta_dma16(a_base + (size_t)wa.a_slab * a_slab_bytes, a_off[q], lds + stage * STAGE + (q * NP + pw) * 256);
-      wa.advance();
+      wa.advance_kept(kym, kxm);
     };
     issue_a(0, 0);
     if (S > 1) issue_a(1, 1);
     const int pl = p.pool;
     const ta_pixel_walk walk(p, pl ? pt0 >> 2 : pt0, HoWo);
     const int in_ch = p.in_ch_off + (p.group_cout ? (ct0 / p.group_cout) * p.group_cin : 0);
-    const size_t off0 = (size_t)walk.img0 * p.in_img + (size_t)((walk.y0 << pl) * p.stride) * p.in_row +
-                        (size_t)((walk.x0 << pl) * p.stride) * p.in_pix + p.in_off0 + in_ch;
+    const size_t off0 = p.in_base0 ? (size_t)(p.in_off0 + in_ch)
+                                   : (size_t)walk.img0 * p.in_img + (size_t)((walk.y0 << pl) * p.stride) * p.in_row +
+                                         (size_t)((walk.x0 << pl) * p.stride) * p.in_pix + p.in_off0 + in_ch;
     const char* b_base = (const char*)(p.in + off0);
     ta_k_walk wb(p, s_begin);
+    wb.seek_kept(kym, kxm);
 #pragma unroll
     for (int q = QA; q < NI; ++q) {
       const int d = (q * NP + pw) * 8 + (lane >> 3) - BN;
@@ -124,11 +144,11 @@
       b_off[q - QA] = (unsigned)((off - off0) * 4 + lchunk * 16);
       ta_dma16(b_base + wb.b_off, b_off[q - QA], lds + (q * NP + pw) * 256);
     }
-    wb.advance();
+    wb.advance_kept(kym, kxm);
     auto issue_b = [&](int stage) {
 #pragma unroll
       for (int q = QA; q < NI; ++q) ta_dma16(b_base + wb.b_off, b_off[q - QA], lds + stage * STAGE + (q * NP + pw) * 256);
-      wb.advance();
+      wb.advance_kept(kym, kxm);
     };
     if (wave == NC) TA_STAMP(9);
     if (S > 1) issue_b(1);
@@ -500,14 +520,28 @@
   const long long grid = (long long)g.groups * 8 * q.k_split;
   q.fast_div = (grid < (1 << 24) && (long long)q.M + BM < (1 << 24)) ? 1 : 0;
   const long long n_img = q.Ho * q.Wo > 0 ? ((long long)q.M + q.Ho * q.Wo - 1) / (q.Ho * q.Wo) : 0;
-  auto fits = [&](long long img_stride, int off0) { return ((n_img + 1) * img_stride + off0) * 4 < (1LL << 32); };
-  bool ok = lean_ok && q.out_fmt == split_fmt && (q.cout & 7) == 0 && ((q.out_ch | q.res_ch | q.o2_ch) & 7) == 0 && fits(q.out_img, q.out_off0);
-  if (q.res) ok = ok && q.res_fmt == split_fmt && fits(q.res_img, q.res_off0);
-  if (q.out2) ok = ok && q.o2_fmt == split_fmt && fits(q.o2_img, q.o2_off0);
+  auto fits = [&](long long img_stride, long long row_stride, long long pix_stride, int off0) {
+    const long long extent = std::max((n_img + 1) * img_stride, n_img * img_stride + (long long)q.Ho * row_stride + (long long)q.Wo * pix_stride);
+    return (extent + off0) * 4 < (1LL << 32);
+  };
+  bool ok = lean_ok && q.out_fmt == split_fmt && (q.cout & 7) == 0 && ((q.out_ch | q.res_ch | q.o2_ch) & 7) == 0 && fits(q.out_img, q.out_row, q.out_pix, q.out_off0);
+  if (q.res) ok = ok && q.res_fmt == split_fmt && fits(q.res_img, q.res_row, q.res_pix, q.res_off0);
+  if (q.out2) ok = ok && q.o2_fmt == split_fmt && fits(q.o2_img, q.o2_row, q.o2_pix, q.o2_off0);
   const bool plain = !q.res && !q.out2;
   ok = ok && (q.pool ? (plain && q.act == TA_ACT_RELU) : (q.bias9 ? (plain && q.act == TA_ACT_PRELU) : (plain || (q.res && q.act == TA_ACT_NONE))));
   q.fast_drain = ok ? 1 : 0;
   if (ok) ctx->conv_counts[TA_CV_COUNT - 1] += 1;
+}
+
+static void split_skip_facts(ta_ctx* ctx, ta_conv_launch& q, int BM) {
+  const bool ok = q.skip_n > 0 && q.stride == 1 && q.uniform_k && !q.pool && q.k_split == 1 && !q.bias9 && q.fast_div && q.k_h <= 32 && q.k_w <= 32 &&
+                  q.n_slabs == q.k_w * q.k_h * q.k_cblocks && q.Ho == q.skip_h && q.Wo == (long long)q.skip_w * q.skip_n;
+  if (!ok) q.skip_n = 0;
+  q.skip_rn = q.skip_n ? 1.0f / (float)q.skip_n : 0.f;
+  if (ctx->slab_counting) {
+    ctx->slabs_full += (int64_t)((q.M + BM - 1) / BM) * q.n_slabs;
+    ctx->slabs_run += ta_tap_tile_slabs(q, BM);
+  }
 }
 
 template <int CM, int CN, int NP, int PREC, int STAGES>
@@ -520,6 +554,9 @@
   ta_conv_launch q = p;
   constexpr int SPLIT_FMT = PREC == PREC_F16 ? TA_FMT_F16 : (prec_half(PREC) ? TA_FMT_SPLIT16 : TA_FMT_SPLIT);
   split_launch_facts(ctx, q, g, BM, SPLIT_FMT, PREC != PREC_F32 && p.k_split == 1);
+  split_skip_facts(ctx, q, BM);
+  if (q.in_base0 && ((long long)q.in_off0 + q.M / (q.Ho * q.Wo) * (long long)q.in_img + (long long)(q.Ho + q.k_h) * q.in_row + (long long)(q.Wo + q.k_w) * q.in_pix) * 4 >= (1LL << 32))
+    return ta_fail(ctx, TA_E_INVALID, "conv: a batch-innermost input tensor over 4 GiB; split the batch");
   TA_NOTE_KERNEL(ctx, "conv_igemm_split<%d,%d,%d,%d,%d>", CM, CN, NP, PREC, STAGES);
   hipLaunchKernelGGL(kern, dim3(g.groups * 8 * p.k_split), dim3(64 * (CM * CN + NP)), lds_bytes, ctx->stream, q);
   TA_HIP(ctx, hipGetLastError());
diff --git a/terran_amd/csrc/model_load.hip b/terran_amd/csrc/model_load.hip
--- a/terran_amd/csrc/model_load.hip
+++ b/terran_amd/csrc/model_load.hip
@@ -49,8 +49,15 @@
   memcpy(ops.data(), (const char*)blob + h.ops_off, h.n_ops * sizeof(ta_op_desc));
   auto bad_w = [&](int64_t off, size_t need) { return off >= 0 && (uint64_t)off + need > (uint64_t)h.weights_bytes; };
 
+  out->batch_inner.assign(T, 0);
   for (int t = 0; t < T; ++t) {
+    if (td[t].fmt >= 0 && (td[t].fmt & ~255) == TA_TENSOR_BATCH_INNER) {
+      out->batch_inner[t] = 1;
+      td[t].fmt &= 255;
+    }
     const ta_tensor_desc& d = td[t];
+    if (out->batch_inner[t] && (d.alias_of != -1 || t == h.input_tensor))
+      return no("model blob: tensor %d: a batch-innermost tensor is neither the input nor a view", t);
     if (!within(d.channels, 1, MAX_DIM) || !within(d.halo, 0, 1024) || !within(d.alias_of, -2, T - 1) || d.alias_of == t)
       return no("model blob: malformed tensor %d", t);
     if ((d.fmt != TA_FMT_F32 && d.channels % 32) || (d.fmt == TA_FMT_F16 && d.channels % 64) || d.fmt < 0 || d.fmt > TA_FMT_F16)
@@ -58,8 +65,12 @@
     if (d.unscale_off >= 0 && (t == h.input_tensor || (d.unscale_off & 3) || bad_w(d.unscale_off, (size_t)d.channels * sizeof(float))))
       return no("model blob: inconsistent activation scales (tensor %d)", t);
   }
-  for (int i = 0; i < h.n_outputs; ++i)
+  for (int i = 0; i < h.n_outputs; ++i) {
     if (!within(h.outputs[i], 0, T - 1)) return no("model blob: output %d is tensor %d, out of range", i, h.outputs[i]);
+    if (out->batch_inner[h.outputs[i]]) return no("model blob: output %d is a batch-innermost tensor", i);
+  }
+  for (int t = 0; t < T; ++t)
+    if (td[t].alias_of >= 0 && out->batch_inner[td[t].alias_of]) return no("model blob: tensor %d views a batch-innermost tensor", t);
 
   std::vector<char> set(T, 0);
   set[h.input_tensor] = 1;
@@ -124,6 +135,14 @@
     if (why) return no("model blob: malformed op %d: %s", oi, why);
 
     const ta_tensor_desc &ti = td[op.in], &to = td[op.out];
+    {
+      const std::vector<char>& bi = out->batch_inner;
+      const bool touches = bi[op.in] || bi[op.out] || (op.res >= 0 && bi[op.res]) || (op.out2 >= 0 && bi[op.out2]);
+      if (touches && (op.type != TA_OP_CONV || op.stride != 1 || op.pool || (op.res >= 0 && bi[op.res]) || (op.out2 >= 0 && bi[op.out2]) ||
+                      ta_op_border_bias(op) || ta_op_lane(op) ||
+                      (bi[op.in] && (ti.fmt != ta_split_fmt_of(op.prec) || !ta_conv_k_geometry(op, ti.fmt).uniform || op.n_slabs < 2))))
+        return no("model blob: op %d: a batch-innermost tensor outside a chain of plain stride-1 convs", oi);
+    }
     if (!view_ready(op.in)) return no("model blob: alias tensor %d used before its source %d (op %d)", op.in, ti.alias_of, oi);
     if (!set[op.in]) return no("model blob: op %d reads unset tensor %d", oi, op.in);
     if (op.type != TA_OP_CONV && (ti.fmt == TA_FMT_F16 || to.fmt == TA_FMT_F16))
diff --git a/terran_amd/csrc/model_plan.hip b/terran_amd/csrc/model_plan.hip
--- a/terran_amd/csrc/model_plan.hip
+++ b/terran_amd/csrc/model_plan.hip
@@ -127,6 +127,7 @@
       ts[i].unscale_host = m->unscale_host[i].data();
     }
     ts[i].n = n;
+    ts[i].bi = m->batch_inner[i] && n % 32 == 0;
   }
   TA_TRY(infer_shapes(m, h, w, ts, set));
 
diff --git a/terran_amd/csrc/model_run.hip b/terran_amd/csrc/model_run.hip
--- a/terran_amd/csrc/model_run.hip
+++ b/terran_amd/csrc/model_run.hip
@@ -146,6 +146,26 @@
         }
         p.variant = ta_op_forced_variant(op);
         if (ta_op_border_bias(op)) p.bias9 = wptr(m, op.scale2_off);
+        const bool view = ti.bi && to.bi;
+        if (ti.bi || to.bi) {
+          if (m->run_n != pl.n) return ta_fail(ctx, TA_E_INVALID, "conv: a batch-innermost plan of %d images run with %d", pl.n, m->run_n);
+          if (view) {
+            p.Wo = to.w * pl.n;
+            p.in_pix = ti.cf();
+            p.tap_pix = pl.n * ti.cf();
+            p.in_img = (int)((size_t)ti.hp() * ti.wp() * pl.n * ti.cf());
+            p.out_pix = to.cf();
+            p.out_img = (int)((size_t)to.hp() * to.wp() * pl.n * to.cf());
+          } else if (ti.bi) {
+            p.in_base0 = 1;
+          }
+        }
+        if (op.stride == 1 && op.pad > 0 && op.kh * op.kw > 1 && !op.pool && !p.bias9) {
+          p.skip_n = view ? pl.n : 1;
+          p.skip_h = ti.h;
+          p.skip_w = ti.w;
+          p.skip_pad = op.pad;
+        }
         p.range_check = (m->has_half_ops && (m->tensor_read[op.out] || (op.out2 >= 0 && m->tensor_read[op.out2]))) ? 1 : 0;
         p.amax_index = (m->amax_on && oi < TA_AMAX_OPS) ? (int)oi : -1;
         double flops = 2.0 * op.macs_per_pixel * (double)p.M;
diff --git a/terran_amd/csrc/ta_internal.h b/terran_amd/csrc/ta_internal.h
--- a/terran_amd/csrc/ta_internal.h
+++ b/terran_amd/csrc/ta_internal.h
@@ -42,6 +42,8 @@
   int32_t fmt;
   int32_t unscale_off;
 };
+
+#define TA_TENSOR_BATCH_INNER 256
 
 struct ta_op_desc {
   int32_t type;
@@ -132,6 +134,8 @@
   int conv_trace_block = 0;
 #endif
   int64_t conv_counts[16] = {0};
+  bool slab_counting = false;
+  int64_t slabs_full = 0, slabs_run = 0;
   int* range_flag = nullptr;
   int* range_flag_host = nullptr;
   const void* amax_owner = nullptr;
@@ -229,11 +233,15 @@
   const float* unscale_dev = nullptr;
   const float* unscale_host = nullptr;
   bool owns = true;
+  bool bi = false;
   int hp() const { return h + 2 * halo; }
   int wp() const { return w + 2 * halo; }
   size_t elems() const { return (size_t)n * hp() * wp() * c; }
   int cf() const { return ta_fmt_is_half(fmt) ? c / 2 : c; }
-  size_t off(int img, int y, int x) const { return (((size_t)img * hp() + y + halo) * wp() + x + halo) * cf(); }
+  size_t off(int img, int y, int x) const {
+    if (bi) return ((((size_t)y + halo) * wp() + x + halo) * n + img) * cf();
+    return (((size_t)img * hp() + y + halo) * wp() + x + halo) * cf();
+  }
 };
 
 struct ta_strides {
@@ -241,6 +249,7 @@
 };
 static inline ta_strides ta_tensor_strides(const ta_tensor& t, int pad, bool count_c) {
   const int s = count_c ? t.c : t.cf(), sh = t.halo - pad;
+  if (t.bi) return {s, t.wp() * t.n * s, t.n * s, (int)(((size_t)sh * t.wp() + sh) * t.n * s)};
   return {(int)((size_t)t.hp() * t.wp() * s), t.wp() * s, s, (int)(((size_t)sh * t.wp() + sh) * s)};
 }
 
@@ -258,6 +267,10 @@
   int M, Ho, Wo, n_slabs, coutp, cout, act, stride, prec;
   int uniform_k, k_cblocks, k_w, k_h, in_ch_off;
   int in_img, in_row, in_pix, in_off0;
+  int tap_pix;
+  int in_base0;
+  int skip_n, skip_h, skip_w, skip_pad;
+  float skip_rn;
   int out_img, out_row, out_pix, out_off0, out_ch, out_fmt;
   int res_img, res_row, res_pix, res_off0, res_up2, res_ch, res_fmt;
   int o2_img, o2_row, o2_pix, o2_off0, o2_ch, o2_fmt;
@@ -355,6 +368,7 @@
   ta_blob_header hdr;
   std::vector<ta_tensor_desc> tdesc;
   std::vector<ta_op_desc> ops;
+  std::vector<char> batch_inner;
 };
 int ta_program_parse(int kind, const void* blob, size_t bytes, ta_program* out, char* msg, size_t msg_capacity);
 
diff --git a/terran_amd/lib.py b/terran_amd/lib.py
--- a/terran_amd/lib.py
+++ b/terran_amd/lib.py
@@ -119,6 +119,8 @@
     'ta_debug_range_check': (c_int, [c_void_p]),
     'ta_debug_conv_counts': (c_int, [c_void_p, c_void_p, c_int]),
     'ta_debug_kernel_work': (c_int, [c_void_p, C.c_char_p, c_size_t, c_int]),
+    'ta_debug_conv_slabs': (c_int, [c_void_p, c_void_p, c_int, c_int]),
+    'ta_debug_tap_masks': (c_int, [c_int] * 9 + [c_void_p]),
 }
 
 GALLERY_ROW_TILE, GALLERY_QUERY_GROUP, GALLERY_MAX_K = 128, 32, 16
@@ -396,6 +398,14 @@
     rc = lib.ta_program_check(int(kind), blob, len(blob), err, len(err))
     if rc != OK:
         raise TerranAmdError(rc, err.value.decode(errors='replace'))
+
+
+def tap_masks(images, h, w, n, pad, kh, kw, pt0, bm):
+    m = np.zeros(2, np.uint32)
+    rc = load().ta_debug_tap_masks(int(images), int(h), int(w), int(n), int(pad), int(kh), int(kw), int(pt0), int(bm), ptr(m))
+    if rc <= 0:
+        raise TerranAmdError(E_INVALID, 'tap_masks: bad geometry')
+    return int(m[0]), int(m[1])
 
 
 def check_jpeg_options(quality, subsampling):
@@ -611,6 +621,11 @@
             out['lean_epilogue'] = int(c[15])
         return out
 
+    def conv_slabs(self, enable=None, reset=False):
+        c = np.zeros(2, np.int64)
+        self.check(self.lib.ta_debug_conv_slabs(self.h, ptr(c), -1 if enable is None else int(bool(enable)), int(reset)))
+        return int(c[0]), int(c[1])
+
     def kernel_work(self, reset=False):
         buf = C.create_string_buffer(1 << 16)
         self.check(self.lib.ta_debug_kernel_work(self.h, buf, len(buf), int(reset)))
diff --git a/terran_amd/pack/__init__.py b/terran_amd/pack/__init__.py
--- a/terran_amd/pack/__init__.py
+++ b/terran_amd/pack/__init__.py
@@ -1,5 +1,6 @@
 from .arcface import pack_arcface
 from .layout import (ACT_NONE, ACT_PRELU, ACT_RELU, BLOB_VERSION, FMT_F16, FMT_F32, FMT_SPLIT, FMT_SPLIT16, HEADER_DT, MAGIC,
+                     TENSOR_BATCH_INNER,
                      MODEL_ARCFACE, MODEL_OPENPOSE, MODEL_RETINAFACE, OP_CONV, OP_COPYCH, OP_DT, OP_DWCONV, OP_DWPW, OP_MAXPOOL,
                      OP_RFSTEM, PRECISIONS, SPLIT_FMT, TENSOR_DT, fold_input_affine, row_exponents, split_bf16_rows, split_f16_rows)
 from .moments import _ACT_TARGET_LOG2, _CH_SPREAD, act_moments
diff --git a/terran_amd/pack/layout.py b/terran_amd/pack/layout.py
--- a/terran_amd/pack/layout.py
+++ b/terran_amd/pack/layout.py
@@ -14,6 +14,7 @@
 })
 TENSOR_DT = np.dtype([('channels', '<i4'), ('halo', '<i4'), ('alias_of', '<i4'), ('fmt', '<i4'), ('unscale_off', '<i4')])
 FMT_F32, FMT_SPLIT, FMT_SPLIT16, FMT_F16 = 0, 1, 2, 3
+TENSOR_BATCH_INNER = 256
 _OP_I32 = ['type', 'in', 'out', 'in_ch_off', 'cin', 'out_ch_off', 'cout', 'coutp', 'kh', 'kw', 'stride', 'pad',
            'act', 'res', 'res_ch_off', 'res_up2', 'out2', 'out2_ch_off', 'n_slabs', 'prec', 'groups', 'variant', 'pool', 'wscale_log2']
 _OP_I64 = ['w_off', 'bias_off', 'prelu_off', 'scale2_off', 'shift2_off', 'wus_off']
diff --git a/terran_amd/pack/openpose.py b/terran_amd/pack/openpose.py
--- a/terran_amd/pack/openpose.py
+++ b/terran_amd/pack/openpose.py
@@ -55,6 +55,8 @@
         kw = dict(ch_pos=cat_pos, cin_p=OP_XCH) if cin == 185 else dict(in_ch_off=OP_FEAT)
         cur = P.tensor(c1 + c2, l1[1][3] // 2)
         P.conv(xin, cur, W, b, act=ACT_RELU if r1 else ACT_NONE, **kw)
+        if k == 7:
+            P.mark_batch_inner(cur)
         for li in range(1, len(l1) - 1):
             (na, cin, cout, k, relu), (nb, cin2, cout2, k2, relu2) = l1[li], l2[li]
             assert (cin, cout, k, relu) == (cin2, cout2, k2, relu2) and cin % 32 == 0 and cout % 128 == 0
@@ -62,6 +64,8 @@
             b = np.concatenate([np.asarray(sd['model%d_%d.%s.bias' % (st, br, n)]) for br, n in ((1, na), (2, nb))])
             o = P.tensor(2 * cout, l1[li + 1][3] // 2)
             P.conv(cur, o, W, b, act=ACT_RELU if relu else ACT_NONE, groups=2)
+            if k == 7:
+                P.mark_batch_inner(o)
             cur = o
         (np_, cin, co1, k, r1), (nh, cin2, co2, k2, r2) = l1[-1], l2[-1]
         if r1 == r2 and cin == cin2 <= 128:
diff --git a/terran_amd/pack/program.py b/terran_amd/pack/program.py
--- a/terran_amd/pack/program.py
+++ b/terran_amd/pack/program.py
@@ -5,7 +5,7 @@
 
 from . import moments, storage
 from .layout import (ACT_NONE, ACT_RELU, BLOB_VERSION, FMT_F16, HEADER_DT, MAGIC, OP_CONV, OP_DT, OP_DWCONV, OP_DWPW, OP_MAXPOOL,
-                     OP_RFSTEM, PRECISIONS, TENSOR_DT, WeightRegion, _rup, fold_input_affine, op_desc, pack_rows)
+                     OP_RFSTEM, PRECISIONS, TENSOR_BATCH_INNER, TENSOR_DT, WeightRegion, _rup, fold_input_affine, op_desc, pack_rows)
 from .moments import ChannelStats, act_bound, act_moments
 
 
@@ -27,6 +27,7 @@
         self.input_tensor = None
         self.outputs = []
         self.f32_only = set()
+        self.batch_inner = set()
         self.allow_split = True
         self.lane = 0
         self.stats = {}
@@ -44,6 +45,9 @@
         if name:
             self.names[name] = (tid, 0, channels)
         return tid
+
+    def mark_batch_inner(self, tid):
+        self.batch_inner.add(tid)
 
     def tap(self, name, tid, ch_off, ch):
         self.names[name] = (tid, ch_off, ch)
@@ -278,7 +282,7 @@
         for i, (c, h, a) in enumerate(self.tensors):
             unscale_off = self.w.add(_pow2(-scales[i])) if np.any(scales[i] != 0) else -1
             assert unscale_off < 2 ** 31
-            tens[i] = (c, h, a, fmts[i], unscale_off)
+            tens[i] = (c, h, a, fmts[i] | (TENSOR_BATCH_INNER if i in self.batch_inner else 0), unscale_off)
         return tens
 
     @staticmethod
```

New measurement: 1863 frames/s. -17.8%, worse.
